# amzn/pecos

Measured on AMD Instinct MI355X. Metric: XLinear queries/sec @ beam=10 top-k=10; P@1 vs reference; 1/2/4/8 GPU, higher is better.
Workload: dtype f32; 1 GPU; amazon-670k synthetic x1.0: N=490000 D=135000 L=670091 tree=[2, 32, 512, 8192, 670091] nnz/row=75.4 beam=10 topk=10 pp=l3-hinge bias=1.0; parallelism=query-shard x1

## Files before the change

pecos_amd/csrc/xrl_abi.cpp:

```cpp
#include <algorithm>
#include <cstring>
#include <memory>
#include <mutex>

#include "xrl_host_pipeline.h"

namespace xrl {
thread_local std::string g_err;
thread_local bool g_has_err = false;
thread_local int g_device = 0;

void set_err(const std::string& s) { g_err = s; g_has_err = true; }

Model* as_model(void* p) {
    if (!p) fail("null model handle");
    return static_cast<Model*>(p);
}

void use_device(int dev) { XRL_HIP(hipSetDevice(dev)); }

void require_gpu() {
    int n = 0;
    if (hipGetDeviceCount(&n) != hipSuccess || n <= 0)
        fail("libxrl_amd: no HIP device visible -- this library has no CPU fallback");
}

void upload_x(const HostX& x, DevBuf& ptr, DevBuf& idx, DevBuf& val, QueriesDev& d) {
    if (!x.given) fail("null X");
    const uint64_t elems = x.elems();
    if (x.csr) {
        ptr.upload_raw(x.row_ptr, ((size_t)x.rows + 1) * 8);
        idx.upload_raw(x.col_idx, elems * 4);
    }
    val.upload_raw(x.val, elems * 4);
    d = device_view(x, ptr, idx, val);
}
}

using namespace xrl;

extern "C" {

const char* xrl_last_error(void) { return g_has_err ? g_err.c_str() : nullptr; }
void xrl_clear_error(void) { g_has_err = false; }
const char* xrl_version(void) { return "xrl_amd 0.1 (gfx950)"; }

int xrl_device_count(void) {
    int n = 0;
    if (hipGetDeviceCount(&n) != hipSuccess) return 0;
    return n;
}

int xrl_set_device(int device) {
    return guarded_value(-1, [&] { use_device(device); g_device = device; return 0; });
}

static void* load_handle(const char* model_path, int kind, int weight_matrix_type) {
    return guarded_value((void*)nullptr, [&]() -> void* {
        if (!model_path) fail("null model path");
        require_gpu();
        use_device(g_device);
        auto m = kind == 0 ? load_model_from_disk(model_path, weight_matrix_type) : load_mmap_model_from_disk(model_path);
        m->device = g_device; m->src_path = model_path; m->src_kind = kind;
        warm_handle(*m);
        return m.release();
    });
}

void* c_xlinear_load_model_from_disk_ext(const char* model_path, int weight_matrix_type) { return load_handle(model_path, 0, weight_matrix_type); }
void* c_xlinear_load_model_from_disk(const char* model_path) { return load_handle(model_path, 0, 2 ); }
void* c_xlinear_load_mmap_model_from_disk(const char* model_path, const bool) { return load_handle(model_path, 1, 2); }

void c_xlinear_compile_mmap_model(const char* model_path, const char* mmap_model_path) {
    guarded([&] {
        if (!model_path || !mmap_model_path) fail("null path");
        compile_mmap_model(model_path, mmap_model_path);
    });
}

void c_xlinear_destruct_model(void* ptr) {
    guarded([&] {
        if (!ptr) return;
        Model* m = static_cast<Model*>(ptr);
        (void)hipSetDevice(m->device);
        delete m;
    });
}

uint32_t c_xlinear_get_int_attr(void* ptr, const char* attr) {
    uint32_t v = 0;
    guarded([&] {
        Model& m = *as_model(ptr);
        if (!attr) fail("null attr");
        if (!std::strcmp(attr, "depth")) v = (uint32_t)m.layers.size();
        else if (!std::strcmp(attr, "nr_features")) v = m.nr_features;
        else if (!std::strcmp(attr, "nr_labels")) v = m.nr_labels;
        else if (!std::strcmp(attr, "nr_codes")) v = m.nr_codes;
        else if (!std::strcmp(attr, "device")) v = (uint32_t)m.device;
        else if (!std::strcmp(attr, "nr_pred_cols")) {
            const Layer& last = *m.layers.back();
            v = last.reordered ? last.c_rows : last.w_cols;
        }
        else if (!std::strcmp(attr, "nr_bucket_layers")) {
            for (auto& l : m.layers) v += l->dev.bucket ? 1u : 0u;
        }
        else if (!std::strcmp(attr, "nr_bitmap64_layers")) {
            for (auto& l : m.layers) v += l->dev.bitmap64 ? 1u : 0u;
        }
        else if (!std::strcmp(attr, "nr_dense_layers")) {
            for (auto& l : m.layers) v += l->dev.wd ? 1u : 0u;
        }
        else if (!std::strcmp(attr, "merged01")) v = m.layers[0]->dev.wd01 ? 1u : 0u;
        else if (!std::strcmp(attr, "nr_devices")) v = 1u + (uint32_t)m.replicas.size();
        else fail(std::string(attr) + " is not implemented in get_int_attr.");
    });
    return v;
}

int c_xlinear_get_layer_type(void* ptr, int layer_depth) {
    int v = -1;
    guarded([&] {
        Model& m = *as_model(ptr);
        if (layer_depth < 0 || (size_t)layer_depth >= m.layers.size()) fail("layer_depth out of range");
        v = m.weight_matrix_type;
    });
    return v;
}

void c_xlinear_predict_csr_f32(void* ptr, const ScipyCsrF32* input_x, const uint32_t overridden_beam_size,
                               const char* overridden_post_processor_str, const uint32_t overridden_only_topk,
                               const int , py_sparse_allocator_t pred_alloc) {
    guarded([&] { predict_host(ptr, HostX(input_x), overridden_beam_size, overridden_post_processor_str, overridden_only_topk, pred_alloc); });
}

void c_xlinear_predict_drm_f32(void* ptr, const ScipyDrmF32* input_x, const uint32_t overridden_beam_size,
                               const char* overridden_post_processor_str, const uint32_t overridden_only_topk,
                               const int , py_sparse_allocator_t pred_alloc) {
    guarded([&] { predict_host(ptr, HostX(input_x), overridden_beam_size, overridden_post_processor_str, overridden_only_topk, pred_alloc); });
}

int xrl_inspect_model(const char* model_path, uint64_t* out, uint32_t cap) {
    int depth = -1;
    guarded([&] {
        if (!model_path) fail("null model path");
        const std::string path(model_path);
        const JsonValue meta = parse_json_file(path + "/param.json");
        const JsonValue* dv = meta.get("depth");
        if (!dv || dv->type != JsonValue::NUMBER) fail(path + "/param.json: missing \"depth\"");
        const int d_n = (int)dv->num;
        for (int d = 0; d < d_n; ++d) {
            const std::string lp = path + "/" + std::to_string(d) + ".model";
            (void)parse_json_file(lp + "/param.json");
            HostCsc W, C;
            load_csc_npz(lp + "/W.npz", W);
            uint64_t c_rows = W.cols, c_cols = 1, c_nnz = W.cols;
            if (!(d == 0 && !file_exists(lp + "/C.npz"))) { load_csc_npz(lp + "/C.npz", C); c_rows = C.rows; c_cols = C.cols; c_nnz = C.nnz(); }
            const uint64_t rec[6] = {W.rows, W.cols, W.nnz(), c_rows, c_cols, c_nnz};
            for (int i = 0; i < 6; ++i) if (out && (uint32_t)(6 * d + i) < cap) out[6 * d + i] = rec[i];
        }
        depth = d_n;
    });
    return depth;
}

static void* queries_upload(void* model, const HostX& x) {
    return guarded_value((void*)nullptr, [&]() -> void* {
        Model& m = *as_model(model);
        use_device(m.device);
        auto q = std::make_unique<Queries>();
        QueriesDev d{};
        upload_x(x, q->ptr, q->idx, q->val, d);
        set_view(*q, m.device, d);
        return q.release();
    });
}
void* xrl_queries_upload_csr(void* model, const ScipyCsrF32* X) { return queries_upload(model, HostX(X)); }
void* xrl_queries_upload_drm(void* model, const ScipyDrmF32* X) { return queries_upload(model, HostX(X)); }

void* xrl_queries_from_device_csr(void* model, uint32_t rows, uint32_t cols, const uint64_t* d_row_ptr, const uint32_t* d_col_idx,
                                  const float* d_val, uint64_t nnz) {
    return guarded_value((void*)nullptr, [&]() -> void* {
        Model& m = *as_model(model);
        if (rows && (!d_row_ptr || (nnz && (!d_col_idx || !d_val)))) fail("xrl_queries_from_device_csr: null device pointer");
        auto q = std::make_unique<Queries>();
        set_view(*q, m.device, csr_view(rows, cols, d_row_ptr, d_col_idx, d_val, nnz));
        return q.release();
    });
}

void* xrl_queries_tfidf_device(void* model, uint32_t rows, uint32_t cols, const uint64_t* d_row_ptr, const uint32_t* d_col_idx,
                               const float* d_count, uint64_t nnz, const float* d_idf, int binary, int sublinear_tf, int norm_p, float* d_out,
                               void* hip_stream) {
    return guarded_value((void*)nullptr, [&]() -> void* {
        Model& m = *as_model(model);
        if (rows && (!d_row_ptr || (nnz && (!d_col_idx || !d_count)))) fail("xrl_queries_tfidf_device: null device pointer");
        use_device(m.device);
        auto q = std::make_unique<Queries>();
        if (!d_out) q->val.reserve(nnz * 4);
        float* dst = d_out ? d_out : q->val.as<float>();
        hipStream_t s = hip_stream ? static_cast<hipStream_t>(hip_stream) : m.stream;
        DevBuf d_err; d_err.reserve(4);
        XRL_HIP(hipMemsetAsync(d_err.p, 0, 4, s));
        launch_tfidf_weight(d_row_ptr, d_col_idx, d_count, d_idf, rows, cols, binary, sublinear_tf, norm_p, dst, s, 1, 0, d_err.as<uint32_t>());
        uint32_t err = 0;
        XRL_HIP(hipMemcpyAsync(&err, d_err.p, 4, hipMemcpyDeviceToHost, s));
        XRL_HIP(hipStreamSynchronize(s));
        if (err) fail("xrl_queries_tfidf_device: a column id outside [0, cols) (the reference's idx_idf.at() throws)");
        set_view(*q, m.device, csr_view(rows, cols, d_row_ptr, d_col_idx, dst, nnz));
        return q.release();
    });
}

void* xrl_queries_from_device_drm(void* model, uint32_t rows, uint32_t cols, const float* d_val) {
    return guarded_value((void*)nullptr, [&]() -> void* {
        Model& m = *as_model(model);
        if (rows && cols && !d_val) fail("xrl_queries_from_device_drm: null device pointer");
        auto q = std::make_unique<Queries>();
        set_view(*q, m.device, dense_view(rows, cols, d_val));
        return q.release();
    });
}

static void* concat_csr(void* model, uint32_t rows, uint32_t sparse_cols, const uint64_t* d_row_ptr, const uint32_t* d_col_idx, const float* d_val,
                        uint64_t nnz, uint32_t dense_cols, const float* d_emb, int normalize_emb, void* hip_stream) {
    Model& m = *as_model(model);
    if (rows && (!d_row_ptr || (nnz && (!d_col_idx || !d_val)) || (dense_cols && !d_emb))) fail("xrl_queries_concat_device: null device pointer");
    use_device(m.device);
    auto q = std::make_unique<Queries>();
    const uint64_t out_nnz = nnz + (uint64_t)rows * dense_cols;
    q->ptr.reserve(((size_t)rows + 1) * 8); q->idx.reserve(out_nnz * 4); q->val.reserve(out_nnz * 4);
    hipStream_t s = hip_stream ? static_cast<hipStream_t>(hip_stream) : m.stream;
    launch_concat_csr(d_row_ptr, d_col_idx, d_val, d_emb, rows, sparse_cols, dense_cols, normalize_emb, q->ptr.as<uint64_t>(), q->idx.as<uint32_t>(),
                      q->val.as<float>(), s);
    XRL_HIP(hipStreamSynchronize(s));
    set_own_csr(*q, m.device, rows, sparse_cols + dense_cols, out_nnz);
    return q.release();
}

void* xrl_queries_concat_device(void* model, uint32_t rows, uint32_t sparse_cols, const uint64_t* d_row_ptr, const uint32_t* d_col_idx,
                                const float* d_val, uint64_t nnz, uint32_t dense_cols, const float* d_emb, void* hip_stream) {
    return xrl_queries_concat_device_ex(model, rows, sparse_cols, d_row_ptr, d_col_idx, d_val, nnz, dense_cols, d_emb, 0, hip_stream);
}

void* xrl_queries_concat_device_ex(void* model, uint32_t rows, uint32_t sparse_cols, const uint64_t* d_row_ptr, const uint32_t* d_col_idx,
                                   const float* d_val, uint64_t nnz, uint32_t dense_cols, const float* d_emb, int normalize_emb, void* hip_stream) {
    return guarded_value((void*)nullptr, [&] {
        return concat_csr(model, rows, sparse_cols, d_row_ptr, d_col_idx, d_val, nnz, dense_cols, d_emb, normalize_emb, hip_stream);
    });
}

void* xrl_queries_concat_handle(void* model, void* queries, uint32_t dense_cols, const float* d_emb, int normalize_emb, void* hip_stream) {
    return guarded_value((void*)nullptr, [&] {
        if (!queries) fail("xrl_queries_concat_handle: null query handle");
        const QueriesDev& X = static_cast<Queries*>(queries)->dev;
        if (X.dense) fail("xrl_queries_concat_handle: the query handle must hold a CSR");
        return concat_csr(model, X.rows, X.cols, X.row_ptr, X.col_idx, X.val, X.nnz, dense_cols, d_emb, normalize_emb, hip_stream);
    });
}

int xrl_queries_info(void* queries, uint64_t* out4) {
    return guarded_value(-1, [&] {
        if (!queries || !out4) fail("null argument");
        const Queries* q = static_cast<const Queries*>(queries);
        out4[0] = q->dev.rows; out4[1] = q->dev.cols; out4[2] = q->dev.dense ? (uint64_t)q->dev.rows * q->dev.cols : q->dev.nnz; out4[3] = q->dev.dense ? 1 : 0;
        return 0;
    });
}

int xrl_queries_download(void* queries, uint64_t* row_ptr, uint32_t* col_idx, float* val) {
    return guarded_value(-1, [&] {
        if (!queries || !val) fail("null argument");
        const Queries* q = static_cast<const Queries*>(queries);
        XRL_HIP(hipSetDevice(q->device));
        XRL_HIP(hipDeviceSynchronize());
        if (q->dev.dense) {
            XRL_HIP(hipMemcpy(val, q->dev.val, (size_t)q->dev.rows * q->dev.cols * 4, hipMemcpyDeviceToHost));
        } else {
            if (!row_ptr || (q->dev.nnz && !col_idx)) fail("null argument");
            XRL_HIP(hipMemcpy(row_ptr, q->dev.row_ptr, ((size_t)q->dev.rows + 1) * 8, hipMemcpyDeviceToHost));
            if (q->dev.nnz) {
                XRL_HIP(hipMemcpy(col_idx, q->dev.col_idx, (size_t)q->dev.nnz * 4, hipMemcpyDeviceToHost));
                XRL_HIP(hipMemcpy(val, q->dev.val, (size_t)q->dev.nnz * 4, hipMemcpyDeviceToHost));
            }
        }
        return 0;
    });
}

void xrl_queries_free(void* queries) {
    guarded([&] {
        if (!queries) return;
        Queries* q = static_cast<Queries*>(queries);
        (void)hipSetDevice(q->device);
        delete q;
    });
}

static int predict_device_entry(const char* what, bool ranged, void* model, void* queries, uint32_t beam_size, const char* post_processor,
                                uint32_t only_topk, uint32_t* d_out_idx, float* d_out_val, uint32_t* d_out_cnt, uint32_t out_stride,
                                void* hip_stream, int sync, uint32_t row_begin = 0, uint32_t row_count = 0xFFFFFFFFu) {
    return guarded_value(-1, [&] {
        Model& m = *as_model(model);
        if (!queries || !d_out_idx || !d_out_val || !d_out_cnt) fail(std::string(what) + ": null argument");
        std::lock_guard<std::mutex> g(m.mu);
        use_device(m.device);
        const QueriesDev& X = static_cast<Queries*>(queries)->dev;
        PredictOpts o; o.beam_size = beam_size; o.only_topk = only_topk; o.post_processor = post_processor;
        if (ranged) o.reserve_rows = X.rows;
        predict_device(m, X, o, d_out_idx, d_out_val, d_out_cnt, out_stride, static_cast<hipStream_t>(hip_stream), sync != 0, row_begin, row_count);
        return 0;
    });
}

int xrl_predict_device(void* model, void* queries, uint32_t beam_size, const char* post_processor, uint32_t only_topk,
                       uint32_t* d_out_idx, float* d_out_val, uint32_t* d_out_cnt, uint32_t out_stride,
                       void* hip_stream, int sync) {
    return predict_device_entry("xrl_predict_device", false, model, queries, beam_size, post_processor, only_topk, d_out_idx, d_out_val, d_out_cnt, out_stride, hip_stream, sync);
}

int xrl_predict_device_rows(void* model, void* queries, uint32_t beam_size, const char* post_processor, uint32_t only_topk,
                            uint32_t* d_out_idx, float* d_out_val, uint32_t* d_out_cnt, uint32_t out_stride,
                            void* hip_stream, int sync, uint32_t row_begin, uint32_t row_count) {
    return predict_device_entry("xrl_predict_device_rows", true, model, queries, beam_size, post_processor, only_topk, d_out_idx, d_out_val, d_out_cnt, out_stride, hip_stream, sync, row_begin, row_count);
}

int xrl_ensemble_device(int device, uint32_t n_models, uint32_t rows, const uint32_t* const* d_idx, const float* const* d_val,
                        const uint32_t* const* d_cnt, const uint32_t* in_stride, int mode, const float* threshold, uint32_t only_topk,
                        uint32_t* d_out_idx, float* d_out_val, uint32_t* d_out_cnt, uint32_t out_stride, void* hip_stream, int sync) {
    return guarded_value(-1, [&] {
        const std::string what = "xrl_ensemble_device: ";
        if (!d_idx || !d_val || !d_cnt || !in_stride || !d_out_idx || !d_out_val || !d_out_cnt) fail(what + "null argument");
        if (n_models == 0 || n_models > (uint32_t)kEnsembleMaxModels) fail(what + "n_models must be 1.." + std::to_string(kEnsembleMaxModels) + ", got " + std::to_string(n_models));
        EnsembleArgs A{};
        uint64_t total = 0;
        for (uint32_t m = 0; m < n_models; ++m) {
            if (!d_idx[m] || !d_val[m] || !d_cnt[m]) fail(what + "null device pointer for model " + std::to_string(m));
            A.idx[m] = d_idx[m]; A.val[m] = d_val[m]; A.cnt[m] = d_cnt[m]; A.stride[m] = in_stride[m];
            total += in_stride[m];
        }
        if (total > kEnsembleMaxTotal) fail(what + "the input strides sum to " + std::to_string(total) + ", more than " + std::to_string(kEnsembleMaxTotal));
        if (mode != kEnsembleAverage && mode != kEnsembleFinish && mode != kEnsembleRankAverage) fail(what + "unknown mode " + std::to_string(mode));
        if (mode != kEnsembleFinish && (threshold || only_topk)) fail(what + "threshold and only_topk belong to mode finish");
        const uint64_t longest = mode == kEnsembleFinish && only_topk ? std::min<uint64_t>(total, only_topk) : total;
        if (out_stride < longest) fail(what + "out_stride " + std::to_string(out_stride) + " smaller than the longest possible row, " + std::to_string(longest));
        if (rows == 0) return 0;
        require_gpu();
        use_device(device);
        A.n_models = n_models; A.rows = rows; A.mode = mode;
        A.has_threshold = threshold ? 1 : 0; A.threshold = threshold ? *threshold : 0.0f; A.only_topk = only_topk;
        A.out_idx = d_out_idx; A.out_val = d_out_val; A.out_cnt = d_out_cnt; A.out_stride = out_stride;
        hipStream_t s = static_cast<hipStream_t>(hip_stream);
        void* mm = nullptr;
        if (mode == kEnsembleRankAverage) XRL_HIP(hipMallocAsync(&mm, sizeof(uint32_t), s));
        try { launch_ensemble(A, static_cast<uint32_t*>(mm), s); }
        catch (...) { if (mm) (void)hipFreeAsync(mm, s); throw; }
        if (mm) XRL_HIP(hipFreeAsync(mm, s));
        if (sync) XRL_HIP(hipStreamSynchronize(s));
        return 0;
    });
}

int xrl_predict_selected_device(void* model, void* queries, const char* post_processor, const uint32_t* d_sel_idx, const uint32_t* d_sel_cnt,
                                uint32_t sel_stride, uint32_t* d_out_idx, float* d_out_val, uint32_t* d_out_cnt, uint32_t out_stride,
                                uint32_t* d_status, void* hip_stream, int sync) {
    return guarded_value(-1, [&] {
        const std::string what = "xrl_predict_selected_device: ";
        if (!model || !queries || !d_sel_idx || !d_out_idx || !d_out_val || !d_out_cnt) fail(what + "null argument");
        Model& m = *as_model(model);
        const Queries& q = *static_cast<Queries*>(queries);
        if (sel_stride == 0 || sel_stride > kSelectMaxStride) fail(what + "sel_stride must be 1.." + std::to_string(kSelectMaxStride) + ", got " + std::to_string(sel_stride) + " (the host entry point serves longer rows)");
        if (out_stride < sel_stride) fail(what + "out_stride " + std::to_string(out_stride) + " smaller than sel_stride " + std::to_string(sel_stride));
        if (q.device != m.device) fail(what + "the queries live on device " + std::to_string(q.device) + ", the model on device " + std::to_string(m.device));
        std::lock_guard<std::mutex> g(m.mu);
        try { check_selected_inputs(m, q.dev); }
        catch (const Error& e) { fail(what + e.what()); }
        if (q.dev.rows == 0) return 0;
        use_device(m.device);
        predict_selected_device(m, q.dev, post_processor, d_sel_idx, d_sel_cnt, sel_stride, d_out_idx, d_out_val, d_out_cnt, out_stride, d_status,
                                static_cast<hipStream_t>(hip_stream), sync != 0);
        return 0;
    });
}

int xrl_predict_stats(void* model, void* queries, uint32_t beam_size, const char* post_processor, uint32_t only_topk,
                      double* stats_out, uint32_t stats_cap) {
    return guarded_value(-1, [&] {
        Model& m = *as_model(model);
        if (!queries || !stats_out) fail("xrl_predict_stats: null argument");
        if (stats_cap < kStatsPerLayer * m.layers.size()) fail("xrl_predict_stats: stats_out too small (need 8*depth doubles)");
        std::lock_guard<std::mutex> g(m.mu);
        if (m.constrained) fail("xrl_predict_stats: not available while an output constraint is set (the constrained route runs none of the counted kernels)");
        use_device(m.device);
        if (!m.ws) m.ws = std::make_unique<Workspace>();
        const QueriesDev& X = static_cast<Queries*>(queries)->dev;
        const uint32_t k = effective_topk(m, only_topk);
        Workspace& ws = *m.ws;
        ws.out_idx.reserve((size_t)X.rows * k * 4); ws.out_val.reserve((size_t)X.rows * k * 4); ws.out_cnt.reserve((size_t)X.rows * 4);
        PredictOpts o; o.beam_size = beam_size; o.only_topk = only_topk; o.post_processor = post_processor; o.stats_out = stats_out;
        const bool was = m.profiling; m.profiling = false;
        predict_device(m, X, o, ws.out_idx.as<uint32_t>(), ws.out_val.as<float>(), ws.out_cnt.as<uint32_t>(), k, m.stream, true);
        m.profiling = was;
        return 0;
    });
}

static int set_constraint_entry(const char* what, void* model, const uint32_t* labels, uint64_t n, bool on_device, void* hip_stream) {
    return guarded_value(-1, [&] {
        Model& m = *as_model(model);
        std::lock_guard<std::mutex> g(m.mu);
        use_device(m.device);
        set_output_constraint(m, labels, n, on_device, static_cast<hipStream_t>(hip_stream), what);
        return 0;
    });
}

int xrl_set_output_constraint(void* model, const uint32_t* labels, uint64_t n) {
    return set_constraint_entry("xrl_set_output_constraint", model, labels, n, false, nullptr);
}

int xrl_set_output_constraint_device(void* model, const uint32_t* d_labels, uint64_t n, void* hip_stream) {
    return set_constraint_entry("xrl_set_output_constraint_device", model, d_labels, n, true, hip_stream);
}

int xrl_clear_output_constraint(void* model) {
    return guarded_value(-1, [&] {
        Model& m = *as_model(model);
        std::lock_guard<std::mutex> g(m.mu);
        use_device(m.device);
        clear_output_constraint(m);
        return 0;
    });
}

int xrl_output_constraint_info(void* model, uint64_t* out, uint32_t cap) {
    return guarded_value(-1, [&] {
        Model& m = *as_model(model);
        std::lock_guard<std::mutex> g(m.mu);
        const uint32_t n = 1u + (uint32_t)m.layers.size();
        for (uint32_t i = 0; i < n && i < cap && out; ++i) {
            if (i == 0) { out[0] = m.constrained ? 1 : 0; continue; }
            const Layer& L = *m.layers[i - 1];
            out[i] = L.view.active ? L.view.kept : L.n_children;
        }
        return (int)n;
    });
}

int xrl_debug_output_constraint_view(void* model, uint32_t layer, uint32_t* chunk_col_out, uint64_t chunk_col_cap, uint32_t* perm_inv_out, uint64_t perm_inv_cap) {
    return guarded_value(-1, [&] {
        Model& m = *as_model(model);
        if (layer >= m.layers.size()) fail("xrl_debug_output_constraint_view: layer out of range");
        std::lock_guard<std::mutex> g(m.mu);
        const Layer& L = *m.layers[layer];
        if (!L.view.active) return 0;
        use_device(m.device);
        XRL_HIP(hipDeviceSynchronize());
        const uint64_t n_cc = std::min<uint64_t>(chunk_col_cap, (uint64_t)L.dev.n_parents + 1), n_pi = std::min<uint64_t>(perm_inv_cap, L.view.kept);
        if (chunk_col_out && n_cc) XRL_HIP(hipMemcpy(chunk_col_out, L.view.d_chunk_col.p, n_cc * 4, hipMemcpyDeviceToHost));
        if (perm_inv_out && n_pi) XRL_HIP(hipMemcpy(perm_inv_out, L.view.d_perm_inv.p, n_pi * 4, hipMemcpyDeviceToHost));
        return 1;
    });
}

uint32_t xrl_effective_topk(void* model, uint32_t only_topk) {
    return guarded_value(0u, [&] { return effective_topk(*as_model(model), only_topk); });
}

void xrl_profile_enable(void* model, int enable) { guarded([&] { as_model(model)->profiling = enable != 0; }); }
void xrl_profile_reset(void* model) { guarded([&] { Model& m = *as_model(model); resolve_profile(m); m.profile.clear(); }); }
uint32_t xrl_profile_get(void* model, xrl_profile_rec_t* out, uint32_t cap) {
    uint32_t n = 0;
    guarded([&] {
        Model& m = *as_model(model);
        resolve_profile(m);
        n = (uint32_t)m.profile.size();
        for (uint32_t i = 0; i < n && i < cap && out; ++i) {
            std::memset(&out[i], 0, sizeof(out[i]));
            std::strncpy(out[i].name, m.profile[i].name.c_str(), sizeof(out[i].name) - 1);
            out[i].layer = m.profile[i].layer; out[i].launches = m.profile[i].launches;
            out[i].ms = m.profile[i].ms;
        }
    });
    return n;
}

uint32_t xrl_debug_split_chunk(const uint64_t* cum, uint32_t n, uint64_t limit) {
    return guarded_value(0u, [&] { if (!cum) fail("null cum"); return split_chunk(cum, n, limit); });
}

uint64_t xrl_debug_layout_rows(const uint32_t* rptr, uint32_t nrows, int align, uint32_t* ext_out) {
    return guarded_value((uint64_t)0, [&] { if (!rptr) fail("null rptr"); return layout_tile_rows(rptr, nrows, align != 0, ext_out); });
}

uint32_t xrl_debug_host_batches(const uint64_t* row_ptr, uint32_t rows, uint32_t cols, int host_batch_mb, uint32_t* rb_out, uint32_t cap) {
    return guarded_value(0u, [&] {
        HostX x; x.given = true; x.csr = row_ptr != nullptr; x.rows = rows; x.cols = cols; x.row_ptr = row_ptr;
        const std::vector<uint32_t> rb = plan_row_batches(x, host_batch_mb, staged_upload(x, 1));
        for (size_t i = 0; i < rb.size() && i < cap && rb_out; ++i) rb_out[i] = rb[i];
        return (uint32_t)rb.size();
    });
}

#define XRL_OPT(name) {#name, &Model::Options::name}
static const struct { const char* name; int Model::Options::*field; } kIntOptions[] = {
    XRL_OPT(k1_group), XRL_OPT(sort_min_tiles), XRL_OPT(sort_rest), XRL_OPT(sort_rest_min), XRL_OPT(prune_mid), XRL_OPT(leaf_fuse), XRL_OPT(tile_rows),
    XRL_OPT(k2_big_min_k), XRL_OPT(qsort), XRL_OPT(qsort_min_parents), XRL_OPT(qsort_min_rows), XRL_OPT(presence), XRL_OPT(adaptive), XRL_OPT(prune),
    XRL_OPT(host_pipeline), XRL_OPT(host_batch_mb), XRL_OPT(host_register), XRL_OPT(overlap_min_rows),
    XRL_OPT(dense_layers), XRL_OPT(k1q_fuse), XRL_OPT(k1g_first), XRL_OPT(k1g_min_items), XRL_OPT(k1g_variant),
    XRL_OPT(k1_wpb), XRL_OPT(k1_lds_pad), XRL_OPT(k1_ablate),
};
#undef XRL_OPT

static void set_option_one(Model& m, const char* key, int64_t value) {
    if (!std::strcmp(key, "max_batch_rows")) { m.opt.max_batch_rows = value; return; }
    if (!std::strcmp(key, "reserve_rows")) {
        if (value < 0 || value > 0x7FFFFFFF) fail("reserve_rows: expected 0 .. 2^31-1");
        std::lock_guard<std::mutex> g(m.mu);
        use_device(m.device);
        if (!m.ws) m.ws = std::make_unique<Workspace>();
        reserve_outputs(m, (uint32_t)value, effective_topk(m, 0));
        return;
    }
    for (const auto& o : kIntOptions)
        if (!std::strcmp(key, o.name)) { m.opt.*o.field = (int)value; if (o.field == &Model::Options::adaptive) m.fb.restage(); return; }
    fail(std::string("unknown option ") + key);
}

int xrl_set_option(void* model, const char* key, int64_t value) {
    return guarded_value(-1, [&] {
        Model& m = *as_model(model);
        if (!key) fail("null key");
        if (!std::strcmp(key, "devices")) {
            if (value < 1 || value > 64) fail("devices: expected 1..64");
            if (m.src_kind < 0 && value > 1) fail("devices: only models loaded from a folder can be replicated");
            std::lock_guard<std::mutex> g(m.mu);
            if (m.constrained && value > 1) fail("devices: the handle carries an output constraint, which replicas do not share (xrl_clear_output_constraint first)");
            int ndev = 0;
            XRL_HIP(hipGetDeviceCount(&ndev));
            m.replicas.clear();
            for (int64_t i = 1; i < value; ++i) {
                const int dev = (m.device + (int)i) % std::max(1, ndev);
                use_device(dev);
                std::unique_ptr<Model> r = m.src_kind == 0 ? load_model_from_disk(m.src_path, m.weight_matrix_type) : load_mmap_model_from_disk(m.src_path);
                r->device = dev;
                r->opt = m.opt;
                m.replicas.push_back(std::move(r));
            }
            use_device(m.device);
        } else {
            set_option_one(m, key, value);
            for (auto& r : m.replicas) set_option_one(*r, key, value);
        }
        return 0;
    });
}

void xrl_debug_k1_phases(unsigned long long* out8, int reset) { guarded([&] { k1_phase_read(out8, reset != 0); }); }

uint32_t xrl_layer_info(void* model, uint32_t layer, uint64_t* out, uint32_t cap) {
    uint32_t n = 0;
    guarded([&] {
        Model& m = *as_model(model);
        if (layer >= m.layers.size()) fail("xrl_layer_info: layer out of range");
        const Layer& L = *m.layers[layer];
        const uint64_t rec[12] = {
            (uint64_t)(L.dev.bucket ? 1 : (L.dev.bitmap64 ? 2 : 0)), L.bk_levels, (uint64_t)(L.dev.wd ? 1 : 0), 1ull << L.dev.d_gp_log2,
            L.dev.d_ld, L.n_tiles, L.nnz, L.dense_bytes, L.w_rows, L.n_children, L.max_tile_cols, L.device_bytes};
        n = 12;
        for (uint32_t i = 0; i < n && i < cap && out; ++i) out[i] = rec[i];
    });
    return n;
}

uint64_t xrl_model_device_bytes(void* model) {
    return guarded_value((uint64_t)0, [&] { return as_model(model)->device_bytes(); });
}

}
```

pecos_amd/csrc/xrl_k0.hip:

```cpp
#include <hip/hip_runtime.h>

#include "xrl_kernels.h"
#include "xrl_items.h"

namespace xrl {

__global__ void __launch_bounds__(256)
k0_prolongate(const uint32_t* __restrict__ chunk_col, const uint32_t* __restrict__ ptile,
              const TileDesc* __restrict__ tiles, uint32_t nrows, uint32_t beam_in, uint32_t item_ranks, uint32_t TT, uint32_t cand_stride,
              int implicit_root, const uint32_t* __restrict__ p_idx, const float* __restrict__ p_val,
              const uint32_t* __restrict__ p_cnt, uint32_t p_stride, uint32_t* __restrict__ cand_off,
              uint32_t* __restrict__ ncand, ItemDesc* __restrict__ items, const uint64_t* __restrict__ x_row_ptr) {
    const uint32_t q = blockIdx.x * 256u + threadIdx.x;
    if (q >= nrows) return;
    uint64_t xb = 0; uint32_t xl = 0;
    if (x_row_ptr) { xb = x_row_ptr[q]; xl = (uint32_t)(x_row_ptr[q + 1] - xb); }
    const uint32_t cnt = implicit_root ? 1u : min(p_cnt[q], beam_in);
    uint32_t off = 0;
    for (uint32_t j = 0; j < beam_in; ++j) {
        ItemDesc* it = items + ((size_t)q * item_ranks + j) * TT;
        uint32_t nt = 0;
        if (j < cnt) {
            const uint32_t parent = implicit_root ? 0u : p_idx[(size_t)q * p_stride + j];
            const float ps = implicit_root ? 1.0f : p_val[(size_t)q * p_stride + j];
            const uint32_t cb = chunk_col[parent], t0 = ptile[parent];
            nt = ptile[parent + 1] - t0;
            cand_off[(size_t)q * beam_in + j] = off;
            if (j < item_ranks)
                for (uint32_t tt = 0; tt < nt; ++tt)
                    it[tt] = make_item(q, t0 + tt, q * cand_stride + off + (tiles[t0 + tt].col_begin - cb), ps, xb, xl);
            off += chunk_col[parent + 1] - cb;
        }
        if (j < item_ranks) for (uint32_t tt = nt; tt < TT; ++tt) it[tt] = make_item(q, kNoTile, 0u, 0.f, 0, 0u);
    }
    ncand[q] = off;
}

void launch_k0_prolongate(const LayerDev& L, const LayerPlan& P, const QueriesDev& X, BeamDev prev, uint32_t* cand_off,
                          uint32_t* ncand, void* items, hipStream_t s, uint32_t item_ranks) {
    if (P.nrows == 0) return;
    if ((uint64_t)P.nrows * P.cand_stride > 0xFFFFFFFFull) fail("k0: candidate buffer exceeds 2^32 floats; lower max_batch_rows");
    hipLaunchKernelGGL(k0_prolongate, dim3((P.nrows + 255) / 256), dim3(256), 0, s, L.chunk_col, L.ptile, L.tiles,
                       P.nrows, P.beam_in, std::min(item_ranks, P.beam_in), L.max_tiles_per_parent, P.cand_stride, P.implicit_root, prev.idx, prev.val,
                       prev.cnt, prev.stride, cand_off, ncand, static_cast<ItemDesc*>(items),
                       X.dense ? nullptr : X.row_ptr + P.row0);
    XRL_LAUNCH_CHECK();
}
size_t k0_item_bytes() { return sizeof(ItemDesc); }

__global__ void __launch_bounds__(256)
k0b_remaining(const uint32_t* __restrict__ chunk_col, const uint32_t* __restrict__ ptile, const TileDesc* __restrict__ tiles,
              uint32_t nrows, uint32_t beam_in, uint32_t first_rank, uint32_t end_rank, uint32_t cand_stride, const uint32_t* __restrict__ p_idx,
              const float* __restrict__ p_val, const uint32_t* __restrict__ p_cnt, uint32_t p_stride, const uint32_t* __restrict__ cand_off,
              const uint32_t* __restrict__ done, ItemDesc* __restrict__ items, uint32_t* __restrict__ n_items,
              const uint64_t* __restrict__ x_row_ptr) {
    const uint32_t q = blockIdx.x * 256u + threadIdx.x;
    const int lane = threadIdx.x & 63;
    const bool live = q < nrows && !done[q];
    const uint32_t cnt = live ? min(min(p_cnt[q], beam_in), end_rank) : 0u;
    uint32_t n = 0;
    for (uint32_t j = first_rank; j < cnt; ++j) { const uint32_t parent = p_idx[(size_t)q * p_stride + j]; n += ptile[parent + 1] - ptile[parent]; }
    uint32_t incl = n;
#pragma unroll
    for (int d = 1; d < 64; d <<= 1) { const uint32_t y = (uint32_t)__shfl_up((int)incl, d, 64); if (lane >= d) incl += y; }
    const uint32_t total = (uint32_t)__shfl((int)incl, 63, 64);
    uint32_t base = 0;
    if (lane == 63 && total) base = atomicAdd(n_items, total);
    base = (uint32_t)__shfl((int)base, 63, 64) + incl - n;
    if (n == 0) return;
    uint64_t xb = 0; uint32_t xl = 0;
    if (x_row_ptr) { xb = x_row_ptr[q]; xl = (uint32_t)(x_row_ptr[q + 1] - xb); }
    for (uint32_t j = first_rank; j < cnt; ++j) {
        const uint32_t parent = p_idx[(size_t)q * p_stride + j];
        const float ps = p_val[(size_t)q * p_stride + j];
        const uint32_t cb = chunk_col[parent], t0 = ptile[parent], nt = ptile[parent + 1] - t0;
        const uint32_t off = cand_off[(size_t)q * beam_in + j];
        for (uint32_t tt = 0; tt < nt; ++tt)
            items[base++] = make_item(q, t0 + tt, q * cand_stride + off + (tiles[t0 + tt].col_begin - cb), ps, xb, xl);
    }
}

void launch_k0b_remaining(const LayerDev& L, const LayerPlan& P, const QueriesDev& X, BeamDev prev, const uint32_t* cand_off, const uint32_t* done,
                          uint32_t first_rank, void* items, uint32_t* n_items, hipStream_t s, uint32_t end_rank) {
    if (P.nrows == 0) return;
    XRL_HIP(hipMemsetAsync(n_items, 0, 4, s));
    hipLaunchKernelGGL(k0b_remaining, dim3((P.nrows + 255) / 256), dim3(256), 0, s, L.chunk_col, L.ptile, L.tiles, P.nrows, P.beam_in, first_rank, end_rank,
                       P.cand_stride, prev.idx, prev.val, prev.cnt, prev.stride, cand_off, done, static_cast<ItemDesc*>(items), n_items,
                       X.dense ? nullptr : X.row_ptr + P.row0);
    XRL_LAUNCH_CHECK();
}

}
```

pecos_amd/csrc/xrl_k1.hip:

```cpp
#include <hip/hip_runtime.h>

#include "xrl_device.h"
#include "xrl_kernels.h"
#include "xrl_items.h"

namespace xrl {

struct K1Args {
    LayerDev L;
    QueriesDev X;
    const ItemDesc* items;
    const uint32_t* n_items;
    float* cand;
    uint64_t n_slots;
    uint32_t row0, acc_stride;
    int pp_kind, pp_p, first_layer;
    int bias_first;
    int ablate;
    uint32_t lds_per_wave;
    uint32_t n_vblocks;
    unsigned long long* phase;
    uint32_t* fb_out;
};

template <int G, int PPC, class ACC>
__device__ __forceinline__ void k1_epilogue(const K1Args& a, const ItemDesc& it, const TileDesc& td, int lig, ACC&& acc_at,
                                            bool add_bias) {
    if (it.tile == kNoTile || (a.ablate & 16)) return;
    float* __restrict__ out = a.cand + it.out_off;
    const float* __restrict__ bp = a.L.bias_prod + td.col_begin;
    if (a.ablate & 8) {
        for (uint32_t c = lig; c < td.ncols; c += G) {
            const float acc = add_bias ? __fadd_rn(acc_at(c), bp[c]) : acc_at(c);
            out[c] = a.first_layer ? acc : pp_combine(a.pp_kind, acc, it.pscore);
        }
        return;
    }
    for (uint32_t c = lig; c < td.ncols; c += G) out[c] = finish_score<PPC>(acc_at(c), add_bias, bp + c, a.pp_kind, a.pp_p, a.first_layer, it.pscore);
}

struct __attribute__((packed, aligned(4))) RowExt { uint32_t start, end; };

template <int G, int NS> struct K1Cfg {
    static constexpr int W = 64 / G;
#ifndef XRL_K1_FEAT
#define XRL_K1_FEAT 64
#endif
    static constexpr int U = (G >= 16) ? XRL_K1_FEAT / G : 8;
    static constexpr int H = (G > 32) ? 2 * G : 64;
    static constexpr int UH = H * NS;
#ifndef XRL_K1_P
#define XRL_K1_P 4
#endif
#ifndef XRL_K1_CLAMP
#define XRL_K1_CLAMP 1
#endif
#ifndef XRL_K1_NB
#define XRL_K1_NB 2
#endif
    static constexpr int P = XRL_K1_P;
    static constexpr int NB = XRL_K1_NB;
    static constexpr int TAIL = (2 * NB - 1) * P;
    static constexpr size_t lds_bytes(uint32_t acc_stride) {
        return (size_t)W * (UH + TAIL) * 8 + (size_t)W * H * 8 + (size_t)W * (acc_stride + G) * 4;
    }
};

#ifndef XRL_K1_WPE
#define XRL_K1_WPE 5
#endif
template <int G, int NS, int PPC, bool DENSE, int LK>
__global__ void __launch_bounds__(256) __attribute__((amdgpu_waves_per_eu(XRL_K1_WPE, 8))) k1_kernel(K1Args a) {
    constexpr int W = K1Cfg<G, NS>::W, H = K1Cfg<G, NS>::H, UH = K1Cfg<G, NS>::UH, P = K1Cfg<G, NS>::P, U = K1Cfg<G, NS>::U,
                  NB = K1Cfg<G, NS>::NB, TAIL = K1Cfg<G, NS>::TAIL;
    extern __shared__ __attribute__((aligned(16))) unsigned char smem_all[];
    const uint32_t wave = threadIdx.x >> 6;
    const uint32_t vblock = blockIdx.x * (blockDim.x >> 6) + wave;
    if (vblock >= a.n_vblocks) return;
    unsigned char* smem = smem_all + (size_t)wave * a.lds_per_wave;
    uint2* uq = reinterpret_cast<uint2*>(smem);
    uint2* hq = reinterpret_cast<uint2*>(uq + W * (UH + TAIL));
    float* acc = reinterpret_cast<float*>(hq + W * H);
    const uint32_t acc_item = a.acc_stride + G;

    const int lane = threadIdx.x & 63;
    const int grp = lane / G, lig = lane % G;
#ifdef XRL_K1_PHASE_PROF
    const bool prof = a.phase != nullptr;
    unsigned long long t_last = prof ? __builtin_readcyclecounter() : 0ull, t_ph[5] = {0, 0, 0, 0, 0};
    auto tick = [&](int ph) { if (prof) { const unsigned long long t = __builtin_readcyclecounter(); t_ph[ph] += t - t_last; t_last = t; } };
#else
    auto tick = [](int) {};
#endif
    ItemDesc it;
    if (!fetch_item<W>(a.items, a.n_items, a.n_slots, a.fb_out, vblock, grp, lane, it)) return;
    const bool active = it.tile != kNoTile;
    TileDesc td{};
    uint64_t xe = 0, cur = 0;
    if (active) {
        td = a.L.tiles[it.tile];
        cur = it.x_begin; xe = it.x_begin + it.x_len;
    }
    const uint32_t* __restrict__ rp = a.L.row_ext + td.rowptr_base;
    const Entry* __restrict__ ent = a.L.entries + td.ent_base;
    float* __restrict__ my_acc = acc + (size_t)grp * acc_item;
    uint2* __restrict__ my_hq = hq + (size_t)grp * H;
    uint2* __restrict__ my_uq = uq + (size_t)grp * (UH + TAIL);
    const uint32_t dummy = a.acc_stride + (uint32_t)lig;
    if (DENSE || a.bias_first) {
        const float* __restrict__ bp = a.L.bias_prod + td.col_begin;
        for (uint32_t c = lig; c < td.ncols; c += G) my_acc[c] = a.L.has_bias ? bp[c] : 0.0f;
    } else if (!(a.ablate & 32)) {
        for (uint32_t c = lig; c < td.ncols; c += G) my_acc[c] = 0.0f;
    }
    wave_sync_lds();
    if (a.ablate & 2) cur = xe;

    const BmWord* __restrict__ bm = a.L.bitmap + (LK != 0 ? 0ull : (uint64_t)(active ? it.tile : 0u) * a.L.nwords);
    const BmWord64* __restrict__ bm64 = a.L.bitmap64 + (LK != 2 ? 0ull : (uint64_t)(active ? it.tile : 0u) * a.L.nwords64);
    const uint32_t* __restrict__ bkt = LK == 1 ? a.L.bucket + (uint64_t)(active ? it.tile : 0u) * (a.L.bk_n + 1u) : nullptr;
    const uint32_t* __restrict__ ridx_t = a.L.row_idx + td.rowptr_base;
    const uint64_t xlast = xe > cur ? xe - 1 : 0;
    uint32_t nh = 0;
    tick(0);

    auto drain = [&]() {
        if (a.ablate & 4) { nh = 0; return; }
        tick(1);
        wave_sync_lds();
        uint32_t nu = 0;
        for (uint32_t h0 = 0; __any(h0 < nh); h0 += G) {
            const uint32_t h = h0 + lig;
            const bool ok = h < nh;
            const uint2 hv = my_hq[ok ? h : 0u];
            const bool need = ok && (LK != 2 || DENSE || (hv.y >> 25) == 0x7Fu);
            const uint32_t s = need ? ((LK == 2 && !DENSE) ? (hv.y & 0x1FFFFFFu) : hv.y) : 0u;
            const uint32_t rl = rp[s];
            const uint32_t rx = need ? rl : hv.y;
            const uint32_t rs = rx & 0x1FFFFFFu;
            const uint32_t len = ok ? (rx >> 25) + 1u : 0u;
            uint32_t cnt = (NS == 1) ? (len ? 1u : 0u) : min((len + G - 1) / G, (uint32_t)NS);
            uint32_t incl = cnt;
            if (G > 1) {
#pragma unroll
                for (int d = 1; d < G; d <<= 1) { const uint32_t y = __shfl_up(incl, d, G); if (lig >= d) incl += y; }
            }
            const uint32_t base = nu + incl - cnt;
#pragma unroll
            for (int k = 0; k < NS; ++k)
                if ((uint32_t)k < cnt) {
                    const uint32_t n_k = (k == NS - 1) ? len - (uint32_t)k * G : min(len - (uint32_t)k * G, (uint32_t)G);
                    my_uq[base + k] = make_uint2(hv.x, (rs + (uint32_t)k * G) | (n_k << 25));
                }
            nu += (G > 1) ? __shfl(incl, G - 1, G) : incl;
        }
        uint32_t nu_max = nu;
#pragma unroll
        for (int d = G; d < 64; d <<= 1) nu_max = max(nu_max, (uint32_t)__shfl_xor((int)nu_max, d, 64));
        nu_max = __builtin_amdgcn_readfirstlane(nu_max);
        for (uint32_t j = nu + lig; j < nu_max + (uint32_t)TAIL; j += G) my_uq[j] = make_uint2(0u, 0u);
        wave_sync_lds();
        tick(2);
        const uint2* __restrict__ uqp = my_uq;
        struct Batch { uint32_t xv[P], cn[P]; Entry e[P]; };
        auto load_batch = [&](const uint2* q, Batch& B) {
            uint32_t st[P];
#pragma unroll
            for (int p = 0; p < P; ++p) { const uint2 d = q[p]; B.xv[p] = d.x; st[p] = d.y & 0x1FFFFFFu; B.cn[p] = d.y >> 25; }
#pragma unroll
            for (int p = 0; p < P; ++p) {
#if XRL_K1_CLAMP
                B.e[p] = ent[st[p] + ((uint32_t)lig < B.cn[p] ? (uint32_t)lig : 0u)];
#else
                B.e[p] = ent[st[p] + (uint32_t)lig];
#endif
            }
        };
        auto apply_batch = [&](const Batch& B) {
#pragma unroll
            for (int p = 0; p < P; ++p) {
                const float v = __uint_as_float(B.xv[p]);
                const uint32_t ci = (uint32_t)lig < B.cn[p] ? B.e[p].col : dummy;
                my_acc[ci] = __fadd_rn(my_acc[ci], __fmul_rn(v, B.e[p].val));
                wave_sync_lds();
            }
        };
        Batch ring[NB];
#pragma unroll
        for (int b = 0; b < NB - 1; ++b) load_batch(uqp + b * P, ring[b]);
        for (uint32_t i0 = 0; i0 < nu_max; i0 += NB * P) {
#pragma unroll
            for (int b = 0; b < NB; ++b) {
                load_batch(uqp + (b + NB - 1) * P, ring[(b + NB - 1) % NB]);
                apply_batch(ring[b]);
            }
            uqp += NB * P;
        }
        nh = 0;
        tick(3);
    };

    if (DENSE) {
        const float* __restrict__ xd = a.X.val + ((uint64_t)a.row0 + it.q) * a.X.cols;
        const uint32_t* __restrict__ ridx = a.L.row_idx + td.rowptr_base;
        uint32_t nr = active ? td.nrows : 0u;
        if (active && td.bias_slot != kNoBias) nr -= 1;
        for (uint32_t s0 = 0; __any(s0 < nr); s0 += H) {
            for (uint32_t j = lig; j < (uint32_t)H; j += G) {
                const uint32_t sidx = s0 + j;
                const bool ok = sidx < nr;
                const uint32_t f = ridx[ok ? sidx : 0u];
                const float xval = xd[f < a.X.cols ? f : 0u];
                if (ok) my_hq[j] = make_uint2(__float_as_uint(f < a.X.cols ? xval : 0.0f), sidx);
            }
            nh = s0 < nr ? min((uint32_t)H, nr - s0) : 0u;
            drain();
        }
        k1_epilogue<G, PPC>(a, it, td, lig, [&](uint32_t c) { return my_acc[c]; }, false);
        return;
    }
    uint32_t skip = 0;
    while (__any(cur < xe)) {
        bool overflow = false;
        {
            uint32_t f[U]; float v[U];
            load_features<G, U>(a.X.col_idx, a.X.val, cur, xe, xlast, a.L.w_rows, lig, f, v);
            bool hit[U]; uint32_t slot[U];
            if (LK == 0) {
                if (a.ablate & 1) {
#pragma unroll
                    for (int u = 0; u < U; ++u) f[u] = 0xFFFFFFFFu;
                }
                probe_bitmap32<U>(bm, f, hit, slot, [](const BmWord& w, uint32_t before) { return w.rank + before; });
            } else if (LK == 2) {
                probe_bitmap64<U>(bm64, f, hit, slot, [](const BmWord64& w, uint32_t before) { return before == 0u ? w.ext0 : (0xFE000000u | (w.rank + before)); });
            } else {
                uint32_t hi[U];
#pragma unroll
                for (int u = 0; u < U; ++u) {
                    const bool inr = f[u] != 0xFFFFFFFFu;
                    const RowExt be = *reinterpret_cast<const RowExt*>(bkt + (inr ? (f[u] >> a.L.bk_shift) : 0u));
                    slot[u] = be.start; hi[u] = inr ? be.end : be.start;
                }
                for (uint32_t lv = a.L.bk_levels; lv > 0; --lv) {
                    const uint32_t stp = 1u << (lv - 1);
#pragma unroll
                    for (int u = 0; u < U; ++u) {
                        const uint32_t np = slot[u] + stp;
                        const bool in = np < hi[u];
                        const uint32_t r = ridx_t[in ? np : slot[u]];
                        slot[u] = (in && r <= f[u]) ? np : slot[u];
                    }
                }
#pragma unroll
                for (int u = 0; u < U; ++u) hit[u] = slot[u] < hi[u] && ridx_t[slot[u]] == f[u];
            }
            overflow = queue_hits<G, U, H>(hit, v, slot, my_hq, grp, lig, nh, skip, cur, xe);
        }
        if (__any(overflow)) drain();
    }
    drain();
    k1_epilogue<G, PPC>(a, it, td, lig, [&](uint32_t c) { return my_acc[c]; }, a.L.has_bias != 0 && !a.bias_first);
#ifdef XRL_K1_PHASE_PROF
    if (prof) {
        tick(4);
        if (lane == 0) { for (int i = 0; i < 5; ++i) atomicAdd(&a.phase[i], t_ph[i]); atomicAdd(&a.phase[5], 1ull); }
    }
#endif
}

template <class KERNEL>
static void launch_k1_any(KERNEL kernel, K1Args a, int W, size_t lds_wave, const K1Tune& tune, hipStream_t s) {
    lds_wave = (lds_wave + (size_t)std::max(0, tune.lds_pad) + 15) & ~(size_t)15;
    int wpb = (tune.wpb == 2 || tune.wpb == 4) ? tune.wpb : 1;
    while (wpb > 1 && lds_wave * wpb > 160 * 1024) wpb >>= 1;
    const size_t lds = lds_wave * wpb;
    if (lds > 160 * 1024) fail("k1: LDS request exceeds 160 KiB");
    if (lds > 48 * 1024)
        XRL_HIP(hipFuncSetAttribute(reinterpret_cast<const void*>(kernel), hipFuncAttributeMaxDynamicSharedMemorySize, (int)lds));
    const uint64_t vblocks = (a.n_slots + W - 1) / W;
    const uint64_t blocks = (vblocks + wpb - 1) / wpb;
    if (vblocks > 0x7FFFFFFFull) fail("k1: grid too large; lower max_batch_rows");
    a.lds_per_wave = (uint32_t)lds_wave; a.n_vblocks = (uint32_t)vblocks;
    hipLaunchKernelGGL(kernel, dim3((uint32_t)blocks), dim3(64 * wpb), lds, s, a);
    XRL_LAUNCH_CHECK();
}

static unsigned long long* g_phase_buf = nullptr;
unsigned long long* k1_phase_buffer() {
    if (!g_phase_buf) { XRL_HIP(hipMalloc(&g_phase_buf, 8 * 8)); XRL_HIP(hipMemset(g_phase_buf, 0, 64)); }
    return g_phase_buf;
}
void k1_phase_read(unsigned long long out[8], bool reset) {
    XRL_HIP(hipDeviceSynchronize());
    XRL_HIP(hipMemcpy(out, k1_phase_buffer(), 64, hipMemcpyDeviceToHost));
    if (reset) XRL_HIP(hipMemset(g_phase_buf, 0, 64));
}

int k1_auto_group(const LayerDev& L, const Layer& host, int dense) {
    (void)host; (void)dense;
    if (L.max_tile_cols <= 8) return 8;
    if (L.max_tile_cols <= 16) return 16;
    return 32;
}

void launch_k1(const LayerDev& L, const LayerPlan& P, const QueriesDev& X, const void* items, const uint32_t* n_items,
               float* cand, int group, hipStream_t s) {
    if (P.nrows == 0) return;
    if ((P.tune.tile_rows >= 2 || (P.tune.tile_rows == 1 && !n_items)) && P.tune.ablate == 0 && k1t_serves(L, X)) { launch_k1t(L, P, X, items, n_items, cand, s); return; }
    K1Args a;
    a.L = L; a.X = X; a.items = static_cast<const ItemDesc*>(items); a.n_items = n_items; a.cand = cand;
    a.n_slots = (uint64_t)P.nrows * P.beam_in * L.max_tiles_per_parent;
    a.row0 = P.row0; a.pp_kind = P.pp.kind; a.pp_p = P.pp.p; a.first_layer = P.first_layer; a.bias_first = P.bias_first;
    a.acc_stride = L.max_tile_cols | 1u;
    const int ablate = P.tune.ablate;
    a.ablate = ablate & 0xFF;
    a.phase = ((ablate & 64) && ((ablate >> 8) == 0 || (ablate >> 8) == P.layer + 1)) ? k1_phase_buffer() : nullptr;
    a.fb_out = (n_items && P.fb_host && P.layer >= 0 && P.layer < kFbLayers) ? P.fb_host + fb_items_word(P.layer) : nullptr;
    const int ppc = pp_class(P.pp);
#define XRL_K1_PP(GG, NN, DD, LL) do { if (ppc) launch_k1_any(&k1_kernel<GG, NN, 1, DD, LL>, a, 64 / GG, lds, P.tune, s); else launch_k1_any(&k1_kernel<GG, NN, 0, DD, LL>, a, 64 / GG, lds, P.tune, s); } while (0)
#define XRL_K1(GG, NN) do { \
        const size_t lds = K1Cfg<GG, NN>::lds_bytes(a.acc_stride); \
        if (X.dense) XRL_K1_PP(GG, NN, true, 0); \
        else if (L.bucket) XRL_K1_PP(GG, NN, false, 1); \
        else if (L.bitmap64) XRL_K1_PP(GG, NN, false, 2); \
        else XRL_K1_PP(GG, NN, false, 0); } while (0)
    if (group < 1 || group > 64 || (group & (group - 1))) fail("k1: lanes-per-item must be a power of two in [1, 64]");
    auto max_ns = [](int g) { return g < 8 ? 1u : (g == 32 ? 4u : 2u); };
    auto units = [&](int g) { return (L.max_tile_cols + (uint32_t)g - 1) / (uint32_t)g; };
    while (group < 64 && units(group) > max_ns(group)) group <<= 1;
    const uint32_t ns = units(group);
    switch (group) {
    case 1: XRL_K1(1, 1); break;
    case 2: XRL_K1(2, 1); break;
    case 4: XRL_K1(4, 1); break;
    case 8: if (ns <= 1) XRL_K1(8, 1); else XRL_K1(8, 2); break;
    case 16: if (ns <= 1) XRL_K1(16, 1); else XRL_K1(16, 2); break;
    case 32: if (ns <= 1) XRL_K1(32, 1); else if (ns == 2) XRL_K1(32, 2); else if (ns == 3) XRL_K1(32, 3); else XRL_K1(32, 4); break;
    default: if (ns <= 1) XRL_K1(64, 1); else XRL_K1(64, 2); break;
    }
#undef XRL_K1
#undef XRL_K1_PP
}

}
```

pecos_amd/csrc/xrl_k1t.hip:

```cpp
#include <hip/hip_runtime.h>

#include <cfloat>
#include <cmath>

#include "xrl_device.h"
#include "xrl_kernels.h"
#include "xrl_items.h"

namespace xrl {

namespace {

struct K1TArgs {
    LayerDev L;
    QueriesDev X;
    const ItemDesc* items;
    const uint32_t* n_items;
    float* cand;
    uint64_t n_slots;
    int pp_kind, pp_p, first_layer, bias_first;
    uint32_t n_vblocks;
    uint32_t* fb_out;
    uint32_t wt_bytes;
    const uint32_t* p_cnt; const float* p_val; uint32_t p_stride, beam_in;
    const uint32_t* xok; const uint32_t* perm_inv;
    uint32_t* out_idx; float* out_val; uint32_t* out_cnt; uint32_t* done;
    uint32_t out_stride, k;
    int mult;
    const uint32_t* p_idx; const uint64_t* x_row_ptr;
    uint32_t cand_stride; uint32_t* cand_off; uint32_t* ncand;
};

template <int NR> struct RowVec;
template <> struct RowVec<1> { float v[1]; };
template <> struct alignas(8) RowVec<2> { float v[2]; };
template <> struct RowVec<3> { float v[3]; };
template <> struct alignas(16) RowVec<4> { float v[4]; };

typedef uint32_t u32x2 __attribute__((ext_vector_type(2)));
typedef uint32_t u32x3 __attribute__((ext_vector_type(3)));
typedef uint32_t u32x4 __attribute__((ext_vector_type(4)));
template <int NR> __device__ __forceinline__ RowVec<NR> row_load_buf(__amdgpu_buffer_rsrc_t rs, uint32_t voff);
template <> __device__ __forceinline__ RowVec<1> row_load_buf<1>(__amdgpu_buffer_rsrc_t rs, uint32_t voff) { return __builtin_bit_cast(RowVec<1>, __builtin_amdgcn_raw_buffer_load_b32(rs, (int)voff, 0, 0)); }
template <> __device__ __forceinline__ RowVec<2> row_load_buf<2>(__amdgpu_buffer_rsrc_t rs, uint32_t voff) { return __builtin_bit_cast(RowVec<2>, __builtin_amdgcn_raw_buffer_load_b64(rs, (int)voff, 0, 0)); }
template <> __device__ __forceinline__ RowVec<3> row_load_buf<3>(__amdgpu_buffer_rsrc_t rs, uint32_t voff) {
    const auto t = __builtin_amdgcn_raw_buffer_load_b96(rs, (int)voff, 0, 0);
    RowVec<3> r; r.v[0] = __uint_as_float(t[0]); r.v[1] = __uint_as_float(t[1]); r.v[2] = __uint_as_float(t[2]); return r;
}
template <> __device__ __forceinline__ RowVec<4> row_load_buf<4>(__amdgpu_buffer_rsrc_t rs, uint32_t voff) { return __builtin_bit_cast(RowVec<4>, __builtin_amdgcn_raw_buffer_load_b128(rs, (int)voff, 0, 0)); }

template <int G, int NR, int PPC, int LK, bool BUF, bool SEL>
__global__ void __launch_bounds__(256) __attribute__((amdgpu_waves_per_eu(5, 8))) k1t_kernel(K1TArgs a) {
    constexpr int W = 64 / G, H = 64, U = (G >= 16) ? 64 / G : 8, UNR = 8, STRIDE = G * NR;
    __shared__ uint2 hq_all[4 * W * (H + UNR)];
    const uint32_t wave = threadIdx.x >> 6;
    const uint32_t vblock = blockIdx.x * 4u + wave;
    if (vblock >= a.n_vblocks) return;
    const int lane = threadIdx.x & 63;
    const int grp = lane / G, lig = lane % G;
    uint2* __restrict__ my_hq = hq_all + ((size_t)wave * W + grp) * (H + UNR);

    auto derive_item = [&](uint64_t q) {
        const uint32_t cnt = min(a.p_cnt[q], a.beam_in);
        const uint32_t parent = cnt ? a.p_idx[q * a.p_stride] : 0u;
        const float ps = a.p_val[q * a.p_stride];
        const uint64_t xb = a.x_row_ptr[q];
        const uint32_t xl = (uint32_t)(a.x_row_ptr[q + 1] - xb);
        const uint32_t t0 = a.L.ptile[parent], t1 = a.L.ptile[parent + 1];
        return make_item((uint32_t)q, (cnt && t1 > t0) ? t0 : kNoTile, (uint32_t)q * a.cand_stride, ps, xb, xl);
    };
    ItemDesc it;
    if (SEL && !a.items && !a.n_items) {
        const uint64_t slot = (uint64_t)vblock * W + grp;
        it = slot < a.n_slots ? derive_item(slot) : make_item(0u, kNoTile, 0u, 0.f, 0, 0u);
    } else if (!fetch_item<W>(a.items, a.n_items, a.n_slots, a.fb_out, vblock, grp, lane, it)) return;
    bool active = it.tile != kNoTile;
    TileDesc td{};
    uint64_t xe = 0, cur = 0, wbase = 0;
    if (active) {
        td = a.L.tiles[it.tile];
        wbase = a.L.wt_base[it.tile];
        cur = it.x_begin; xe = it.x_begin + it.x_len;
    }
    const char* __restrict__ wrow = reinterpret_cast<const char*>(a.L.wt + (BUF ? 0ull : wbase) + (uint32_t)(NR * lig));
    const uint32_t tbase = BUF ? (uint32_t)(wbase * 4ull) : 0u;
    const uint32_t lane_off = (uint32_t)(NR * lig * 4);
    const __amdgpu_buffer_rsrc_t wrs = __builtin_amdgcn_make_buffer_rsrc(const_cast<float*>(a.L.wt), 0, (int)(BUF ? a.wt_bytes : 0u), 0x00020000);
    const uint32_t pad_off = tbase + td.nrows * (uint32_t)(STRIDE * 4);
    float acc[NR];
    {
        const float* __restrict__ bp = a.L.bias_prod + td.col_begin;
#pragma unroll
        for (int k = 0; k < NR; ++k) {
            const uint32_t c = (uint32_t)(NR * lig + k);
            acc[k] = (a.bias_first && a.L.has_bias && c < td.ncols) ? bp[c] : 0.0f;
        }
    }
    const BmWord* __restrict__ bm = a.L.bitmap + (LK != 0 ? 0ull : (uint64_t)(active ? it.tile : 0u) * a.L.nwords);
    const BmWord64* __restrict__ bm64 = a.L.bitmap64 + (LK != 2 ? 0ull : (uint64_t)(active ? it.tile : 0u) * a.L.nwords64);
    const uint64_t xlast = xe > cur ? xe - 1 : 0;
    uint32_t nh = 0;
    bool nonfin = false;

    auto drain = [&](auto exact_tag) {
        constexpr bool EX = decltype(exact_tag)::value;
        wave_sync_lds();
        uint32_t nh_max = nh;
#pragma unroll
        for (int d = G; d < 64; d <<= 1) nh_max = max(nh_max, (uint32_t)__shfl_xor((int)nh_max, d, 64));
        nh_max = __builtin_amdgcn_readfirstlane(nh_max);
        for (uint32_t j = nh + (uint32_t)lig; j < ((nh_max + UNR - 1u) & ~(uint32_t)(UNR - 1)); j += G) my_hq[j] = make_uint2(0u, pad_off);
        wave_sync_lds();
#pragma unroll 1
        for (uint32_t h0 = 0; h0 < nh_max; h0 += UNR) {
            uint2 hv[UNR];
            RowVec<NR> w[UNR];
#pragma unroll
            for (int u = 0; u < UNR; ++u) hv[u] = my_hq[h0 + u];
#pragma unroll
            for (int u = 0; u < UNR; ++u) w[u] = BUF ? row_load_buf<NR>(wrs, hv[u].y + lane_off) : *reinterpret_cast<const RowVec<NR>*>(wrow + hv[u].y);
#pragma unroll
            for (int u = 0; u < UNR; ++u) {
                const float x = __uint_as_float(hv[u].x);
#pragma unroll
                for (int k = 0; k < NR; ++k) {
                    const float s = __fadd_rn(acc[k], __fmul_rn(x, w[u].v[k]));
                    acc[k] = (EX && __float_as_uint(w[u].v[k]) == kMissing) ? acc[k] : s;
                }
            }
        }
        nh = 0;
    };
    auto drain_any = [&]() {
        if (nonfin) drain(std::true_type{}); else drain(std::false_type{});
        nonfin = false;
    };

    uint32_t skip = 0;
    while (__any(cur < xe)) {
        bool overflow = false;
        {
            uint32_t f[U]; float v[U];
            load_features<G, U>(a.X.col_idx, a.X.val, cur, xe, xlast, a.L.w_rows, lig, f, v);
            bool nf = false;
#pragma unroll
            for (int u = 0; u < U; ++u) nf |= (cur + (uint64_t)(u * G + lig) < xe) & ((__float_as_uint(v[u]) & 0x7F800000u) == 0x7F800000u);
            nonfin = nonfin || __any(nf);
            bool hit[U]; uint32_t off[U];
            if (LK == 0) probe_bitmap32<U>(bm, f, hit, off, [&](const BmWord& w, uint32_t before) { return tbase + (w.rank + before) * (uint32_t)(STRIDE * 4); });
            else probe_bitmap64<U>(bm64, f, hit, off, [&](const BmWord64& w, uint32_t before) { return tbase + (w.rank + before) * (uint32_t)(STRIDE * 4); });
            overflow = queue_hits<G, U, H>(hit, v, off, my_hq, grp, lig, nh, skip, cur, xe);
        }
        if (__any(overflow)) drain_any();
    }
    drain_any();

    if constexpr (SEL) {
        static_assert(G == 32, "the selecting epilogue ranks one item per half-wavefront");
        int lane_e = lane;
        asm volatile("" : "+v"(lane_e));
        const int grp = lane_e >> 5, lig = lane_e & 31;
        const uint64_t slot = (uint64_t)vblock * W + grp;
        const bool qv = slot < a.n_slots;
        const uint64_t q = qv ? slot : 0;
        if constexpr (NR == 4) {
            it = a.items ? a.items[q] : derive_item(q);
            active = qv && it.tile != kNoTile;
            td = a.L.tiles[active ? it.tile : 0u];
        }
        const uint32_t pc = a.p_cnt[q], xok = a.xok[q];
        const float ps_next = a.p_val[q * a.p_stride + 1u];
        const float* __restrict__ bp = a.L.bias_prod + td.col_begin;
        const bool add_bias = a.L.has_bias != 0 && !a.bias_first;
        uint32_t key[NR], sb[NR];
#pragma unroll
        for (int k = 0; k < NR; ++k) {
            const uint32_t c = (uint32_t)(NR * lig + k);
            key[k] = 0u; sb[k] = 0u;
            if (active && c < td.ncols) {
                const float v = finish_score<PPC>(acc[k], add_bias, bp + c, a.pp_kind, a.pp_p, a.first_layer, it.pscore);
                sb[k] = __float_as_uint(v); key[k] = score_key(v);
            }
        }
        const bool limited = min(pc, a.beam_in) > 1u;
        const uint32_t thr = score_key(a.mult ? fmaxf(ps_next, 0.0f) : ps_next);
        uint32_t c_lo = 0, c_hi = 0;
#pragma unroll
        for (int k = 0; k < NR; ++k) {
            const unsigned long long b = __ballot(key[k] >= thr);
            c_lo += (uint32_t)__popc((uint32_t)b); c_hi += (uint32_t)__popc((uint32_t)(b >> 32));
        }
        const bool d = !limited || (xok != 0u && ps_next == ps_next && (grp ? c_hi : c_lo) >= a.k);
        if (!a.items && __any(qv && !d)) {
            const uint32_t cnt = min(pc, a.beam_in);
            const bool mine = qv && !d && (uint32_t)lig < cnt;
            uint32_t wd = 0;
            if (mine) { const uint32_t pj = a.p_idx[q * a.p_stride + (uint32_t)lig]; wd = a.L.chunk_col[pj + 1] - a.L.chunk_col[pj]; }
            uint32_t incl = wd;
#pragma unroll
            for (int s = 1; s < 32; s <<= 1) { const uint32_t y = (uint32_t)__shfl_up((int)incl, s, 32); if (lig >= s) incl += y; }
            const uint32_t total = (uint32_t)__shfl((int)incl, 31, 32);
            if (mine) a.cand_off[q * a.beam_in + (uint32_t)lig] = incl - wd;
            if (qv && !d && lig == 0) a.ncand[q] = total;
        }
        if (active && !d) {
            float* __restrict__ out = a.cand + it.out_off;
#pragma unroll
            for (int k = 0; k < NR; ++k) { const uint32_t c = (uint32_t)(NR * lig + k); if (c < td.ncols) out[c] = __uint_as_float(sb[k]); }
        }
        uint32_t osb, ops, kk_lo, kk_hi;
        halfwave_topk_extract<NR>(key, sb, a.k, lane_e, osb, ops, kk_lo, kk_hi);
        const uint32_t kk = grp ? kk_hi : kk_lo;
        if (qv) {
            if ((uint32_t)lig < kk) {
                uint32_t child = td.col_begin + ops;
                if (a.perm_inv) child = a.perm_inv[child];
                a.out_idx[q * a.out_stride + (uint32_t)lig] = child;
                a.out_val[q * a.out_stride + (uint32_t)lig] = __uint_as_float(osb);
            }
            if (lig == 0) { a.out_cnt[q] = kk; a.done[q] = d ? 1u : 0u; }
        }
        return;
    }
    if (!active) return;
    float* __restrict__ out = a.cand + it.out_off;
    const float* __restrict__ bp = a.L.bias_prod + td.col_begin;
    const bool add_bias = a.L.has_bias != 0 && !a.bias_first;
#pragma unroll
    for (int k = 0; k < NR; ++k) {
        const uint32_t c = (uint32_t)(NR * lig + k);
        if (c < td.ncols) out[c] = finish_score<PPC>(acc[k], add_bias, bp + c, a.pp_kind, a.pp_p, a.first_layer, it.pscore);
    }
}

__global__ void __launch_bounds__(256)
tile_rows_kernel(const TileDesc* __restrict__ tiles, const uint32_t* __restrict__ row_ext, const Entry* __restrict__ entries,
                 const uint64_t* __restrict__ wt_base, uint32_t stride, uint32_t* __restrict__ wt) {
    const TileDesc td = tiles[blockIdx.x];
    uint32_t* __restrict__ dst = wt + wt_base[blockIdx.x];
    const uint32_t* __restrict__ ext = row_ext + td.rowptr_base;
    const Entry* __restrict__ ent = entries + td.ent_base;
    const uint32_t sub = threadIdx.x >> 5, l = threadIdx.x & 31u;
    for (uint32_t r = sub; r < td.nrows; r += 8u) {
        const uint32_t e = ext[r], start = e & 0x1FFFFFFu, len = (e >> 25) + 1u;
        for (uint32_t i = l; i < len; i += 32u) {
            const Entry x = ent[start + i];
            const uint32_t b = __float_as_uint(x.val);
            dst[(uint64_t)r * stride + x.col] = b == kMissing ? 0u : b;
        }
    }
}

}

void k1t_shape(uint32_t max_tile_cols, int& g, int& nr) {
    g = max_tile_cols <= 8 ? 8 : max_tile_cols <= 16 ? 16 : 32;
    nr = (int)((max_tile_cols + (uint32_t)g - 1) / (uint32_t)g);
    if (nr < 1) nr = 1;
}

void launch_tile_rows(const LayerDev& L, uint64_t total_floats, uint32_t* wt, hipStream_t s) {
    XRL_HIP(hipMemsetD32Async(reinterpret_cast<hipDeviceptr_t>(wt), (int)kMissing, total_floats, s));
    if (L.n_tiles) {
        hipLaunchKernelGGL(tile_rows_kernel, dim3(L.n_tiles), dim3(256), 0, s, L.tiles, L.row_ext, L.entries, L.wt_base, L.wt_stride, wt);
        XRL_LAUNCH_CHECK();
    }
}

bool k1t_serves(const LayerDev& L, const QueriesDev& X) { return L.wt != nullptr && !X.dense && (L.bitmap || L.bitmap64) && !L.bucket; }

bool k1t_selects(const LayerDev& L, const LayerPlan& P, const QueriesDev& X) {
    int g, nr;
    k1t_shape(L.max_tile_cols, g, nr);
    return k1t_serves(L, X) && P.tune.tile_rows >= 1 && P.tune.ablate == 0 && L.max_tiles_per_parent == 1 && g == 32 && nr <= 4 &&
           P.k >= 1 && P.k <= kTopkExtractMaxK && P.beam_in >= 2 && !P.implicit_root && !P.first_layer && k2_wave_path(P);
}

void launch_k1t(const LayerDev& L, const LayerPlan& P, const QueriesDev& X, const void* items, const uint32_t* n_items, float* cand, hipStream_t s,
                const K1TSelect* sel) {
    if (P.nrows == 0) return;
    K1TArgs a{};
    a.L = L; a.X = X; a.items = static_cast<const ItemDesc*>(items); a.n_items = n_items; a.cand = cand;
    a.n_slots = sel ? (uint64_t)P.nrows : (uint64_t)P.nrows * P.beam_in * L.max_tiles_per_parent;
    a.pp_kind = P.pp.kind; a.pp_p = P.pp.p; a.first_layer = P.first_layer; a.bias_first = P.bias_first;
    a.fb_out = (n_items && P.fb_host && P.layer >= 0 && P.layer < kFbLayers) ? P.fb_host + fb_items_word(P.layer) : nullptr;
    int g, nr;
    k1t_shape(L.max_tile_cols, g, nr);
    if ((uint32_t)(g * nr) != L.wt_stride || nr > 4) fail("k1t: the layer's tile rows were laid out for another shape");
    const uint64_t vblocks = (a.n_slots + (uint64_t)(64 / g) - 1) / (uint64_t)(64 / g);
    if (vblocks > 0x7FFFFFFFull) fail("k1t: grid too large; lower max_batch_rows");
    a.n_vblocks = (uint32_t)vblocks;
    const int ppc = pp_class(P.pp);
    const int lk = L.bitmap64 ? 2 : 0;
    const bool buf = L.wt_bytes != 0 && L.wt_bytes < 0xFFFFFF00ull;
    a.wt_bytes = buf ? (uint32_t)L.wt_bytes : 0u;
    if (sel) {
        if (n_items || !k1t_selects(L, P, X)) fail("k1t: the selecting epilogue does not serve this launch");
        if (!sel->done || !sel->xok) fail("k1t: bound pruning needs the done and the per-query guard flags");
        a.p_cnt = sel->prev.cnt; a.p_val = sel->prev.val; a.p_stride = sel->prev.stride; a.beam_in = P.beam_in;
        a.xok = sel->xok; a.perm_inv = L.perm_inv;
        a.out_idx = sel->out.idx; a.out_val = sel->out.val; a.out_cnt = sel->out.cnt; a.done = sel->done;
        a.out_stride = sel->out.stride; a.k = P.k;
        a.mult = (P.pp.kind == PP_SIGMOID || P.pp.kind == PP_LP_HINGE) ? 1 : 0;
        if (!items) {
            if (!sel->cand_off || !sel->ncand || P.beam_in > 32u) fail("k1t: the launch cannot derive its items");
            if ((uint64_t)P.nrows * P.cand_stride > 0xFFFFFFFFull) fail("k1t: candidate buffer exceeds 2^32 floats; lower max_batch_rows");
            a.p_idx = sel->prev.idx; a.x_row_ptr = X.row_ptr + P.row0; a.cand_stride = P.cand_stride; a.cand_off = sel->cand_off; a.ncand = sel->ncand;
        }
    }
    const dim3 grid((a.n_vblocks + 3u) / 4u), block(256);
#define XRL_K1T_L(GG, NN, BB, SS) do { \
        if (ppc) { if (lk) hipLaunchKernelGGL((k1t_kernel<GG, NN, 1, 2, BB, SS>), grid, block, 0, s, a); else hipLaunchKernelGGL((k1t_kernel<GG, NN, 1, 0, BB, SS>), grid, block, 0, s, a); } \
        else     { if (lk) hipLaunchKernelGGL((k1t_kernel<GG, NN, 0, 2, BB, SS>), grid, block, 0, s, a); else hipLaunchKernelGGL((k1t_kernel<GG, NN, 0, 0, BB, SS>), grid, block, 0, s, a); } } while (0)
#define XRL_K1T(GG, NN) do { if (buf) XRL_K1T_L(GG, NN, true, false); else XRL_K1T_L(GG, NN, false, false); } while (0)
#define XRL_K1T_S(NN) do { if (sel) { if (buf) XRL_K1T_L(32, NN, true, true); else XRL_K1T_L(32, NN, false, true); } else XRL_K1T(32, NN); } while (0)
    if (g == 8) XRL_K1T(8, 1);
    else if (g == 16) XRL_K1T(16, 1);
    else if (nr == 1) XRL_K1T_S(1);
    else if (nr == 2) XRL_K1T_S(2);
    else if (nr == 3) XRL_K1T_S(3);
    else XRL_K1T_S(4);
#undef XRL_K1T_S
#undef XRL_K1T
#undef XRL_K1T_L
    XRL_LAUNCH_CHECK();
}

}
```

pecos_amd/csrc/xrl_k2.hip:

```cpp
#include <hip/hip_runtime.h>

#include "xrl_device.h"
#include "xrl_kernels.h"

namespace xrl {

struct K2Args {
    const uint32_t* chunk_col;
    const uint32_t* perm_inv;
    const uint32_t* p_idx; const uint32_t* p_cnt; uint32_t p_stride;
    const uint32_t* cand_off; const uint32_t* ncand; const float* cand;
    uint32_t* out_idx; float* out_val; uint32_t* out_cnt;
    uint32_t nrows, beam_in, cand_stride, k, out_stride;
    int implicit_root;
    const float* p_val;
    int mult;
    uint32_t rank_limit;
    uint32_t* done;
    const uint32_t* skip_done;
    const uint32_t* xok;
};

__device__ __forceinline__ uint32_t k2_child_id(const K2Args& a, uint64_t q, uint32_t pos) {
    uint32_t parent = 0, off = 0;
    if (!a.implicit_root) {
        const uint32_t cnt = min(a.p_cnt[q], a.beam_in);
        uint32_t jj = 0;
        for (uint32_t j = 1; j < cnt; ++j) if (a.cand_off[q * a.beam_in + j] <= pos) jj = j; else break;
        off = a.cand_off[q * a.beam_in + jj];
        parent = a.p_idx[q * a.p_stride + jj];
    }
    const uint32_t child = a.chunk_col[parent] + (pos - off);
    return a.perm_inv ? a.perm_inv[child] : child;
}

__global__ void __launch_bounds__(64) k2_topk_reg(K2Args a) {
    const uint64_t q = blockIdx.x;
    const int lane = threadIdx.x;
    const uint32_t n = a.ncand[q], k = a.k;
    const float* __restrict__ cv = a.cand + q * a.cand_stride;
    float lv = -INFINITY, th = -INFINITY;
    uint32_t lp = 0, m = 0;
    constexpr int KB = 4;
    const uint32_t nlast = n ? n - 1 : 0;
    for (uint32_t base0 = 0; base0 < n; base0 += 64 * KB) {
        float vb[KB];
#pragma unroll
        for (int b = 0; b < KB; ++b) { const uint32_t p = base0 + b * 64 + lane; vb[b] = cv[p < n ? p : nlast]; }
#pragma unroll
        for (int b = 0; b < KB; ++b) {
            const uint32_t base = base0 + b * 64;
            const uint32_t p = base + lane;
            const bool valid = p < n;
            const float v = vb[b];
            unsigned long long mask = __ballot(valid && (m < k || v > th));
            while (mask) {
                const int l = __ffsll((long long)mask) - 1;
                mask &= mask - 1;
                const float vv = __shfl(v, l);
                if (m == k && !(vv > th)) continue;
                const int r = __popcll(__ballot((uint32_t)lane < m && lv >= vv));
                const float uv = __shfl_up(lv, 1);
                const uint32_t up = __shfl_up(lp, 1);
                if (lane > r) { lv = uv; lp = up; }
                else if (lane == r) { lv = vv; lp = base + l; }
                if (m < k) ++m;
                th = (m == k) ? __shfl(lv, (int)k - 1) : -INFINITY;
            }
        }
    }
    if ((uint32_t)lane < m) {
        a.out_idx[q * a.out_stride + lane] = k2_child_id(a, q, lp);
        a.out_val[q * a.out_stride + lane] = lv;
    }
    if (lane == 0) a.out_cnt[q] = m;
}

__global__ void __launch_bounds__(64) k2_topk_lds(K2Args a) {
    extern __shared__ __attribute__((aligned(16))) unsigned char smem[];
    float* lv = reinterpret_cast<float*>(smem);
    uint32_t* lp = reinterpret_cast<uint32_t*>(lv + a.k);
    const uint64_t q = blockIdx.x;
    const int lane = threadIdx.x;
    const uint32_t n = a.ncand[q], k = a.k;
    const float* __restrict__ cv = a.cand + q * a.cand_stride;
    float th = -INFINITY;
    uint32_t m = 0;
    for (uint32_t base = 0; base < n; base += 64) {
        const uint32_t p = base + lane;
        const bool valid = p < n;
        const float v = valid ? cv[p] : 0.f;
        unsigned long long mask = __ballot(valid && (m < k || v > th));
        while (mask) {
            const int l = __ffsll((long long)mask) - 1;
            mask &= mask - 1;
            const float vv = __shfl(v, l);
            if (m == k && !(vv > th)) continue;
            uint32_t r = 0;
            for (uint32_t i0 = 0; i0 < m; i0 += 64) {
                const uint32_t i = i0 + lane;
                r += (uint32_t)__popcll(__ballot(i < m && lv[i] >= vv));
            }
            const uint32_t e = (m < k) ? m : k - 1;
            for (uint32_t hi = e; hi > r;) {
                const uint32_t lo = (hi - r > 64) ? hi - 64 : r;
                const uint32_t i = lo + lane;
                const bool mv = i < hi;
                float tv = 0.f; uint32_t tp = 0;
                if (mv) { tv = lv[i]; tp = lp[i]; }
                wave_sync_lds();
                if (mv) { lv[i + 1] = tv; lp[i + 1] = tp; }
                wave_sync_lds();
                hi = lo;
            }
            if (lane == 0) { lv[r] = vv; lp[r] = base + l; }
            wave_sync_lds();
            if (m < k) ++m;
            th = (m == k) ? lv[k - 1] : -INFINITY;
        }
    }
    wave_sync_lds();
    for (uint32_t i = lane; i < m; i += 64) {
        a.out_idx[q * a.out_stride + i] = k2_child_id(a, q, lp[i]);
        a.out_val[q * a.out_stride + i] = lv[i];
    }
    if (lane == 0) a.out_cnt[q] = m;
}

template <int NS>
__global__ void __launch_bounds__(256) k2_topk_wave(K2Args a) {
    __shared__ uint2 sc_all[4 * 64];
    const int lane = threadIdx.x & 63;
    const uint32_t wave = __builtin_amdgcn_readfirstlane(threadIdx.x >> 6);
    const uint32_t q32 = blockIdx.x * 4u + wave;
    if (q32 >= a.nrows) return;
    const uint64_t q = q32;
    if (a.skip_done && a.skip_done[q]) return;
    uint32_t n = min(a.ncand[q], (uint32_t)(64 * NS));
    const uint32_t bcnt0 = a.implicit_root ? 1u : min(a.p_cnt[q], a.beam_in);
    const uint32_t rl = min(a.rank_limit, a.beam_in - 1u);
    const uint32_t lim_off = a.rank_limit ? a.cand_off[q * a.beam_in + rl] : 0u;
    const float ps_next = a.rank_limit ? a.p_val[q * a.p_stride + rl] : 0.0f;
    const bool limited = a.rank_limit != 0u && bcnt0 > a.rank_limit;
    if (limited) n = min(n, lim_off);
    const float* __restrict__ cv = a.cand + q * a.cand_stride;
    const uint32_t slast = a.cand_stride - 1u;
    const uint32_t bcnt = a.implicit_root ? 1u : min(a.p_cnt[q], a.beam_in);
    const bool lane_beam = !a.implicit_root && bcnt <= 64u;
    uint32_t b_off = 0xFFFFFFFFu, b_par = 0u, b_cc = 0u;
    if (lane_beam && (uint32_t)lane < bcnt) { b_off = a.cand_off[q * a.beam_in + lane]; b_par = a.p_idx[q * a.p_stride + lane]; b_cc = a.chunk_col[b_par]; }
    uint32_t key[NS], sbits[NS], pos[NS];
#pragma unroll
    for (int r = 0; r < NS; ++r) {
        const uint32_t p = (uint32_t)r * 64u + (uint32_t)lane;
        const float v = cv[min(p, slast)];
        sbits[r] = __float_as_uint(v); pos[r] = p;
        key[r] = p < n ? score_key(v) : 0u;
    }
    if (a.done) {
        bool d = true;
        if (limited) d = a.xok[q] != 0u && ps_next == ps_next && wave_count_ge<NS>(key, score_key(a.mult ? fmaxf(ps_next, 0.0f) : ps_next)) >= a.k;
        if (lane == 0) a.done[q] = d ? 1u : 0u;
    }
    uint32_t rank, sb, pp;
    const uint32_t kk = wave_topk<NS>(key, sbits, pos, a.k, sc_all + wave * 64u, lane, rank, sb, pp);
    uint32_t child;
    if (lane_beam) {
        uint32_t jj = 0;
        for (uint32_t j = 1; j < bcnt; ++j) jj = ((uint32_t)__builtin_amdgcn_readlane((int)b_off, (int)j) <= pp) ? j : jj;
        const uint32_t off = (uint32_t)__shfl((int)b_off, (int)jj, 64), cc = (uint32_t)__shfl((int)b_cc, (int)jj, 64);
        child = cc + (pp - off);
        if ((uint32_t)lane < kk && a.perm_inv) child = a.perm_inv[child];
    } else {
        child = (uint32_t)lane < kk ? k2_child_id(a, q, pp) : 0u;
    }
    if ((uint32_t)lane < kk) {
        a.out_idx[q * a.out_stride + rank] = child;
        a.out_val[q * a.out_stride + rank] = __uint_as_float(sb);
    }
    if (lane == 0) a.out_cnt[q] = kk;
}

size_t k2_max_k() { return (160 * 1024) / 8; }

bool k2_wave_path(const LayerPlan& P) { return P.k <= 64 && P.cand_stride <= 64u * 32u; }

void launch_k2_topk(const LayerDev& L, const LayerPlan& P, BeamDev prev, const uint32_t* cand_off,
                    const uint32_t* ncand, const float* cand, BeamDev out, hipStream_t s, uint32_t rank_limit, uint32_t limited_cands,
                    uint32_t* done, const uint32_t* skip_done, const uint32_t* xok) {
    if (P.nrows == 0) return;
    K2Args a;
    a.p_val = prev.val; a.rank_limit = rank_limit; a.done = done; a.skip_done = skip_done; a.xok = xok;
    if (done && !xok) fail("k2: bound pruning needs the per-query guard flags");
    a.mult = (P.pp.kind == PP_SIGMOID || P.pp.kind == PP_LP_HINGE) ? 1 : 0;
    if ((rank_limit || done || skip_done) && !k2_wave_path(P)) fail("k2: bound pruning needs the register top-k path");
    a.chunk_col = L.chunk_col; a.perm_inv = L.perm_inv;
    a.p_idx = prev.idx; a.p_cnt = prev.cnt; a.p_stride = prev.stride;
    a.cand_off = cand_off; a.ncand = ncand; a.cand = cand;
    a.out_idx = out.idx; a.out_val = out.val; a.out_cnt = out.cnt;
    a.nrows = P.nrows; a.beam_in = P.beam_in; a.cand_stride = P.cand_stride; a.k = P.k; a.out_stride = out.stride;
    a.implicit_root = P.implicit_root;
    if (P.k == 0) fail("k2: only_topk / beam_size resolved to 0");
    if (!rank_limit && !done && !skip_done && (P.k > k2_max_k() || (P.tune.k2_big_min_k > 0 && P.k >= (uint32_t)P.tune.k2_big_min_k))) {
        launch_k2_topk_big(L, P, prev, cand_off, ncand, cand, out.idx, out.val, out.cnt, out.stride, s);
        return;
    }
    if (k2_wave_path(P)) {
        const uint32_t ns = ((rank_limit ? std::min(P.cand_stride, std::max(1u, limited_cands)) : P.cand_stride) + 63u) / 64u;
        const dim3 grid((P.nrows + 3u) / 4u), block(256);
        if (ns <= 1) hipLaunchKernelGGL(k2_topk_wave<1>, grid, block, 0, s, a);
        else if (ns <= 2) hipLaunchKernelGGL(k2_topk_wave<2>, grid, block, 0, s, a);
        else if (ns <= 4) hipLaunchKernelGGL(k2_topk_wave<4>, grid, block, 0, s, a);
        else if (ns <= 8) hipLaunchKernelGGL(k2_topk_wave<8>, grid, block, 0, s, a);
        else if (ns <= 13) hipLaunchKernelGGL(k2_topk_wave<13>, grid, block, 0, s, a);
        else if (ns <= 16) hipLaunchKernelGGL(k2_topk_wave<16>, grid, block, 0, s, a);
        else if (ns <= 24) hipLaunchKernelGGL(k2_topk_wave<24>, grid, block, 0, s, a);
        else hipLaunchKernelGGL(k2_topk_wave<32>, grid, block, 0, s, a);
    } else if (P.k <= 64) {
        hipLaunchKernelGGL(k2_topk_reg, dim3(P.nrows), dim3(64), 0, s, a);
    } else {
        const size_t lds = (size_t)P.k * 8;
        if (P.k > k2_max_k()) fail("k2: only_topk/beam_size " + std::to_string(P.k) + " exceeds the device limit " + std::to_string(k2_max_k()));
        if (lds > 48 * 1024)
            XRL_HIP(hipFuncSetAttribute(reinterpret_cast<const void*>(&k2_topk_lds), hipFuncAttributeMaxDynamicSharedMemorySize, (int)lds));
        hipLaunchKernelGGL(k2_topk_lds, dim3(P.nrows), dim3(64), lds, s, a);
    }
    XRL_LAUNCH_CHECK();
}

}
```

pecos_amd/csrc/xrl_kernels.h:

```cpp
#pragma once
#include "xrl_model.h"

namespace xrl {

struct QueriesDev {
    const uint64_t* row_ptr;
    const uint32_t* col_idx;
    const float* val;
    uint32_t rows, cols;
    int dense;
    uint64_t nnz;
};

struct BeamDev {
    uint32_t* idx;
    float* val;
    uint32_t* cnt;
    uint32_t stride;
};

struct K1Tune { int wpb = 1, lds_pad = 0, ablate = 0, k1g_variant = 0, pres_mode = 1, tile_rows = 1, k2_big_min_k = 0; };

struct LayerPlan {
    uint32_t row0, nrows;
    uint32_t beam_in;
    uint32_t k;
    uint32_t cand_stride;
    PostProc pp;
    int first_layer;
    int implicit_root;
    int prune;
    int bias_first;
    int layer;
    K1Tune tune;
    uint32_t* fb_host = nullptr;
    uint32_t* fb_dev = nullptr;
};

void launch_k0_prolongate(const LayerDev& L, const LayerPlan& P, const QueriesDev& X, BeamDev prev, uint32_t* cand_off,
                          uint32_t* ncand, void* items, hipStream_t s, uint32_t item_ranks = 0xFFFFFFFFu );
void launch_k0b_remaining(const LayerDev& L, const LayerPlan& P, const QueriesDev& X, BeamDev prev, const uint32_t* cand_off, const uint32_t* done,
                          uint32_t first_rank, void* items, uint32_t* n_items, hipStream_t s, uint32_t end_rank = 0xFFFFFFFFu);
bool k2_wave_path(const LayerPlan& P);
size_t k0_item_bytes();
void launch_k1(const LayerDev& L, const LayerPlan& P, const QueriesDev& X, const void* items, const uint32_t* n_items,
               float* cand, int group, hipStream_t s);
void launch_sort_items(const LayerDev& L, uint64_t n_slots, const void* items, void* sorted, uint32_t* H,
                       uint32_t* start, hipStream_t s,
                       const uint32_t* n_dev = nullptr);
void launch_sort_queries(BeamDev prev, uint32_t nrows, uint32_t n_keys, uint32_t* H, uint32_t* start, uint32_t* perm, hipStream_t s);
uint32_t qsort_max_keys();
size_t qsort_hist_bytes(uint32_t nrows, uint32_t n_keys);
void launch_step_marker(hipStream_t s);
uint32_t sort_max_tiles();
size_t sort_hist_bytes(uint64_t n_slots, uint32_t n_tiles);
void launch_k2_topk(const LayerDev& L, const LayerPlan& P, BeamDev prev, const uint32_t* cand_off,
                    const uint32_t* ncand, const float* cand, BeamDev out, hipStream_t s,
                    uint32_t rank_limit = 0 , uint32_t limited_cands = 0 ,
                    uint32_t* done = nullptr , const uint32_t* skip_done = nullptr ,
                    const uint32_t* xok = nullptr );
constexpr int kStatsPerLayer = 8;
void launch_stats(const LayerDev& L, const LayerPlan& P, const QueriesDev& X, BeamDev prev, const uint32_t* ncand, const void* items,
                  double* out8, hipStream_t s, uint64_t item_slots = 0 );
void launch_k3_inner_products(const uint64_t* x_ptr, const uint32_t* x_idx, const float* x_val, int x_dense,
                              const uint64_t* w_ptr, const uint32_t* w_idx, const float* w_val, int w_dense,
                              uint32_t dim, uint64_t len, const uint32_t* rows, const uint32_t* cols,
                              float* out, hipStream_t s);

unsigned long long* k1_phase_buffer();
void k1_phase_read(unsigned long long out[8], bool reset);
void launch_k4_selected(const uint64_t* col_ptr, const uint32_t* row_idx, const float* val, uint32_t w_rows, float bias,
                        const QueriesDev& X, const uint32_t* pair_q, const uint32_t* node, const uint32_t* ppos,
                        const uint64_t* prev_off, const float* prev_val, float* out_val, uint64_t n_pairs,
                        const PostProc& pp, int first_layer, hipStream_t s);
uint32_t k1g_cols(const LayerDev& L);
void launch_k1g(const LayerDev& L, const LayerPlan& P, const QueriesDev& X, const void* items_sorted, const uint32_t* start,
                uint32_t* blk_start, const uint32_t* x_ok, float* cand, hipStream_t s);
void launch_xguard(const QueriesDev& X, uint32_t row0, uint32_t nrows, float wmax, uint32_t* ok, hipStream_t s);
void launch_k1c_csc(const LayerDev& L, const uint64_t* col_ptr, const uint32_t* row_idx, const float* val, const LayerPlan& P,
                    const QueriesDev& X, BeamDev prev, const uint32_t* cand_off, const uint32_t* ncand, float* cand, hipStream_t s);
void launch_concat_csr(const uint64_t* in_ptr, const uint32_t* in_idx, const float* in_val, const float* emb, uint32_t rows,
                       uint32_t sparse_cols, uint32_t dense_cols, int normalize_emb, uint64_t* out_ptr, uint32_t* out_idx, float* out_val, hipStream_t s);
void launch_tfidf_weight(const uint64_t* row_ptr, const uint32_t* col_idx, const float* count, const float* idf, uint32_t rows, uint32_t cols,
                         int binary, int sublinear_tf, int norm_p, float* out, hipStream_t s,
                         uint32_t seg_stride = 1, uint32_t seg_off = 0, uint32_t* err = nullptr);
int k1_auto_group(const LayerDev& L, const Layer& host, int dense);
bool k1t_serves(const LayerDev& L, const QueriesDev& X);
struct K1TSelect { BeamDev prev; const uint32_t* xok; BeamDev out; uint32_t* done; uint32_t* cand_off; uint32_t* ncand; };
bool k1t_selects(const LayerDev& L, const LayerPlan& P, const QueriesDev& X);
void launch_k1t(const LayerDev& L, const LayerPlan& P, const QueriesDev& X, const void* items, const uint32_t* n_items, float* cand, hipStream_t s,
                const K1TSelect* sel = nullptr);
uint32_t k1q_regs(const LayerDev& L, uint32_t beam_in, uint32_t k, bool dense_x);
void launch_k1q(const LayerDev* const* Ls, const LayerPlan* Ps, int n, const QueriesDev& X, BeamDev prev, BeamDev out,
                hipStream_t s, float prune_wmax, uint32_t* out_xok = nullptr,
                const uint32_t* qperm = nullptr );
size_t k2_max_k();
void launch_k2_topk_big(const LayerDev& L, const LayerPlan& P, BeamDev prev, const uint32_t* cand_off, const uint32_t* ncand, const float* cand,
                        uint32_t* out_idx, float* out_val, uint32_t* out_cnt, uint32_t out_stride, hipStream_t s);

constexpr int kEnsembleMaxModels = 8;
constexpr uint32_t kEnsembleMaxTotal = 1024;
enum { kEnsembleAverage = 0, kEnsembleFinish = 1, kEnsembleRankAverage = 2 };
struct EnsembleArgs {
    const uint32_t* idx[kEnsembleMaxModels];
    const float* val[kEnsembleMaxModels];
    const uint32_t* cnt[kEnsembleMaxModels];
    uint32_t stride[kEnsembleMaxModels];
    uint32_t n_models, rows;
    int mode;
    int has_threshold;
    float threshold;
    uint32_t only_topk;
    uint32_t* out_idx;
    float* out_val;
    uint32_t* out_cnt;
    uint32_t out_stride;
};
uint32_t ensemble_slots(uint32_t stride_sum);
void launch_ensemble(const EnsembleArgs& A, uint32_t* mm_scratch, hipStream_t s);

constexpr uint32_t kSelectMaxStride = 1024;
constexpr uint32_t kSelectNone = 0xFFFFFFFFu;
enum { kSelectOk = 0, kSelectOutOfRange = 1, kSelectTwice = 2, kSelectNoParent = 3 };
struct SelectTreeLayer {
    const uint32_t* parent;
    const uint32_t* crank;
    uint32_t c_rows, pad;
};
struct SelectPlanArgs {
    const uint32_t* sel_idx; const uint32_t* sel_cnt;
    uint32_t sel_stride;
    uint32_t row0, nrows;
    uint32_t depth, nr_labels;
    const SelectTreeLayer* tree;
    uint32_t* node; uint32_t* ppos; uint32_t* cnt; uint64_t layer_elems, layer_rows;
    uint32_t* out_idx; uint32_t* out_cnt; uint32_t out_stride;
    unsigned long long* status;
};
void launch_select_plan(const SelectPlanArgs& A, hipStream_t s);
struct SelectScoreArgs {
    const uint64_t* col_ptr; const uint32_t* row_idx; const float* val; uint32_t w_rows; float bias;
    const uint32_t* node; uint32_t node_stride;
    const uint32_t* ppos; const uint32_t* cnt;
    const float* prev_val;
    float* out_val; uint32_t out_stride;
    uint32_t row0, nrows, sel_stride;
};
void launch_k4_selected_dev(const SelectScoreArgs& A, const QueriesDev& X, const PostProc& pp, hipStream_t s);

}
```

pecos_amd/csrc/xrl_model.h:

```cpp
#pragma once
#include <memory>
#include <mutex>
#include <string>
#include <vector>

#include "xrl_common.h"
#include "xrl_feedback.h"
#include "xrl_io.h"

namespace xrl {

constexpr uint32_t kMaxTileCols = 128;
constexpr uint32_t kNoBias = 0xFFFFFFFFu;
constexpr uint32_t kMissing = 0x80000000u;

enum PPKind : int { PP_NOOP = 0, PP_SIGMOID = 1, PP_LOG_SIGMOID = 2, PP_LP_HINGE = 3, PP_LOG_LP_HINGE = 4 };
struct PostProc { int kind = PP_NOOP; int p = 0; };
PostProc parse_post_processor(const char* name);

struct TileDesc {
    uint32_t col_begin;
    uint32_t ncols;
    uint32_t nrows;
    uint32_t bias_slot;
    uint64_t rowptr_base;
    uint64_t ent_base;
};

struct Entry { uint32_t col; float val; };
struct BmWord { uint32_t bits; uint32_t rank; };
struct alignas(16) BmWord64 { uint32_t lo, hi, rank, ext0; };
inline uint32_t pack_row_extent(uint32_t start, uint32_t len) { return start | ((len - 1u) << 25); }

struct LayerDev {
    const TileDesc* tiles;
    const uint32_t* ptile;
    const uint32_t* chunk_col;
    const BmWord* bitmap;
    const BmWord64* bitmap64;
    uint32_t nwords64;
    const uint32_t* bucket;
    uint32_t bk_shift, bk_n, bk_levels;
    const uint32_t* row_ext;
    const uint32_t* row_idx;
    const Entry* entries;
    const uint32_t* perm_inv;
    const float* chunk_alg_bytes;
    const float* bias_prod;
    uint32_t n_parents, n_children, n_tiles, nwords, w_rows;
    uint32_t max_tiles_per_parent, max_tile_cols;
    float bias;
    int has_bias;
    const uint32_t* wd;
    uint64_t d_ld;
    uint32_t d_gp_log2;
    uint32_t d_max_tiles;
    const uint32_t* d_ptile;
    const uint32_t* d_tcol;
    int d_sparse_ok;
    const uint32_t* pres;
    uint32_t pres_words;
    int d_full;
    const uint32_t* tile_parent;
    const uint32_t* wd01; uint32_t wd01_c1;
    const float* wt; const uint64_t* wt_base; uint32_t wt_stride; uint64_t wt_bytes;
    int d_regular;
};

struct ConstraintView {
    bool active = false;
    DevBuf d_chunk_col, d_perm_inv;
    std::vector<uint32_t> chunk_sizes_desc;
    uint64_t kept = 0;
    uint64_t cand_bound(uint32_t beam) const;
    void clear() { active = false; d_chunk_col.release(); d_perm_inv.release(); chunk_sizes_desc.clear(); kept = 0; }
};

struct Layer {
    uint32_t w_rows = 0, w_cols = 0, c_rows = 0, c_cols = 0;
    float bias = 0.f;
    float w_absmax = 0.f;
    uint32_t only_topk = 0;
    PostProc pp;
    std::string pp_name;
    bool reordered = false;
    uint32_t n_children = 0;
    uint32_t n_tiles = 0, nwords = 0, max_tiles_per_parent = 0, max_tile_cols = 0, max_chunk_cols = 0;
    uint64_t nnz = 0, total_rows = 0;
    std::vector<uint32_t> chunk_sizes_desc;
    std::vector<uint64_t> h_c_ptr; std::vector<uint32_t> h_c_idx, h_parent;
    std::string w_path; std::shared_ptr<HostCsc> w_host;
    DevBuf d_csc_ptr, d_csc_idx, d_csc_val; bool csc_ready = false;
    DevBuf d_sel_parent, d_sel_crank;
    DevBuf d_tiles, d_ptile, d_chunk_col, d_bitmap, d_row_ptr, d_row_idx, d_entries, d_perm_inv, d_chunk_alg, d_bias_prod;
    DevBuf d_bucket, d_bitmap64;
    DevBuf d_wd, d_dptile, d_dtcol, d_tile_parent, d_pres;
    DevBuf d_wt, d_wt_base;
    uint64_t dense_bytes = 0;
    uint32_t bk_shift = 0, bk_n = 0, bk_levels = 0;
    ConstraintView view;
    LayerDev dev{};
    uint64_t device_bytes = 0;
    uint64_t buffer_bytes() const;
    uint64_t cand_bound(uint32_t beam) const;
    uint64_t cand_bound_kept(uint32_t beam) const { return view.active ? view.cand_bound(beam) : cand_bound(beam); }
};

struct ProfileSlot { std::string name; uint32_t layer; uint32_t launches = 0; double ms = 0; };
struct PendingEvent { hipEvent_t a, b; size_t slot; };

struct LaneWs {
    DevBuf beam_idx[2], beam_val[2], beam_cnt[2];
    DevBuf cand_off, ncand, cand;
    DevBuf items, items_sorted, sort_hist, sort_start;
    DevBuf blk_start, x_ok;
    DevBuf qperm, qsort_hist, qsort_start;
    DevBuf prune_done, prune_cnt;
};
struct Workspace {
    LaneWs lane[2];
    DevBuf stats;
    DevBuf x_ptr, x_idx, x_val;
    DevBuf out_idx, out_val, out_cnt;
    PinnedBuf h_idx, h_val, h_cnt;
    PinnedBuf stage[3];
    PinnedBuf stage_ptr;
    DevBuf init_idx, init_val, init_cnt;
    DevBuf sel_node, sel_ppos, sel_cnt, sel_val[2], sel_status;
};

struct Model {
    int device = 0;
    int weight_matrix_type = 2;
    std::vector<std::unique_ptr<Layer>> layers;
    uint32_t nr_features = 0, nr_labels = 0, nr_codes = 0;
    hipStream_t stream = nullptr;
    hipStream_t aux_stream = nullptr;
    hipEvent_t ws_done = nullptr;
    hipStream_t ws_stream = nullptr;
    hipStream_t copy_stream = nullptr;
    hipStream_t d2h_stream = nullptr;
    std::vector<hipEvent_t> d2h_events;
    std::vector<hipEvent_t> events;
    struct HostLanes { hipEvent_t done[2] = {nullptr, nullptr}; hipStream_t strm[2] = {nullptr, nullptr}; hipEvent_t join = nullptr; } host_lanes;
    std::mutex mu;
    std::unique_ptr<Workspace> ws;
    bool constrained = false;
    bool csc_route = false;
    DevBuf d_wd01;
    DevBuf d_sel_tree; bool sel_tree_ready = false;
    PruneFeedback fb;
    struct Options {
        int k1_group = 0;
        int k1_wpb = 1, k1_lds_pad = 0, k1_ablate = 0;
        int k1g_variant = 0;
        int64_t max_batch_rows = 0;
        int overlap_min_rows = 0;
        int prune = 1;
        int k2_big_min_k = 0;
        int tile_rows = 1;
        int dense_layers = 1;
        int k1q_fuse = 3;
        int k1g_first = 0;
        int k1g_min_items = 16;
        int adaptive = 1;
        int presence = 1;
        int leaf_fuse = 1;
        int prune_mid = 1;
        int sort_rest = 1;
        int sort_rest_min = 32768;
        int qsort = 1;
        int qsort_min_parents = 64, qsort_min_rows = 131072;
        int sort_min_tiles = 0;
        int host_register = 0;
        int host_batch_mb = 12;
        int host_pipeline = 1;
    } opt;
    std::string src_path; int src_kind = -1;
    std::vector<std::unique_ptr<Model>> replicas;
    bool profiling = false;
    std::vector<ProfileSlot> profile;
    std::vector<PendingEvent> pending;
    Model();
    ~Model();
    uint64_t device_bytes() const;
};

uint32_t split_chunk(const uint64_t* cum, uint32_t n, uint64_t limit);
uint64_t layout_tile_rows(const uint32_t* rptr, uint32_t nrows, bool align, uint32_t* ext);

std::unique_ptr<Layer> compile_layer(const HostCsc& W, const HostCsc& C, float bias, uint32_t only_topk,
                                     const std::string& post_processor,
                                     const std::vector<uint32_t>* perm_inv_override = nullptr, uint32_t orig_rows = 0,
                                     bool structure_only = false);
std::unique_ptr<Model> load_model_from_disk(const std::string& path, int weight_matrix_type);
void finalize_model(Model& m);
std::unique_ptr<Model> load_mmap_model_from_disk(const std::string& path);
void compile_mmap_model(const std::string& npz_path, const std::string& mmap_path);
void ensure_device_csc(Layer& L);
void set_output_constraint(Model& m, const uint32_t* labels, uint64_t n, bool on_device, hipStream_t s, const char* what);
void clear_output_constraint(Model& m);
void ensure_device_tree(Model& m);
void k1t_shape(uint32_t max_tile_cols, int& g, int& nr);
void launch_tile_rows(const LayerDev& L, uint64_t total_floats, uint32_t* wt, hipStream_t s);
inline bool k1q_merged01_addressable(uint32_t w_rows) { return ((uint64_t)w_rows + 2) * 256ull < 0xFFFFFFF0ull; }
void launch_merge01(const uint32_t* wd0, uint64_t ld0, uint32_t k0, const uint32_t* wd1, uint64_t ld1, uint32_t c1, uint32_t rows, uint32_t* out, hipStream_t s);
void launch_presence(const uint32_t* wd, uint64_t ld, uint32_t rows, uint32_t gp_log2, uint32_t n_tiles, uint32_t pres_words, uint32_t* pres, hipStream_t s);
void launch_densify(const uint64_t* col_ptr, const uint32_t* row_idx, const float* val, const uint32_t* src_col,
                    const uint32_t* dst_off, uint32_t n_children, uint32_t w_rows, uint64_t ld, uint32_t* wd, hipStream_t s);

}
```

pecos_amd/csrc/xrl_predict.cpp:

```cpp
#include "xrl_predict.h"
#include "xrl_constrain.h"

#include <algorithm>
#include <cstdio>
#include <cstdlib>

namespace xrl {

size_t profile_slot(Model& m, const char* name, uint32_t layer) {
    for (size_t i = 0; i < m.profile.size(); ++i)
        if (m.profile[i].layer == layer && m.profile[i].name == name) return i;
    m.profile.push_back(ProfileSlot{name, layer});
    return m.profile.size() - 1;
}

namespace {

uint32_t k1g_first_slots(const Layer& L, uint32_t beam_in, int forced = 0) {
    if (forced > 0) return (uint32_t)std::max<int64_t>(1, std::min<int64_t>(beam_in > 1 ? (int64_t)beam_in - 1 : 1, forced));
    return (uint32_t)std::max<uint64_t>(1, std::min<uint64_t>(beam_in > 1 ? beam_in - 1 : 1, 64 / std::max<uint64_t>(1, L.cand_bound(1))));
}

struct LayerShape { uint32_t k, beam_in, cand_stride; PostProc pp; };

enum RouteKind { ROUTE_CSC, ROUTE_K1G, ROUTE_K1Q, ROUTE_TILE, ROUTE_CONSTRAINED };
struct Route {
    RouteKind kind;
    size_t last;
    bool sorted_last;
    int mode;
    int group;
    bool pruned;
    uint32_t J;
    uint32_t stage_end[3]; int n_stage;
    bool fuse, fuse_k0;
    bool sorts_rest;
};

struct Batch {
    Model& m; const Model::Options& opt; const QueriesDev& X; const PredictOpts& o; const std::vector<LayerShape>& shape;
    BeamDev result{}; uint32_t beam_stride = 1;
    bool has_init = false, csc = false, stats = false; double* stats_dev = nullptr;
    uint64_t nb = 1; int lanes = 1;
    PruneFeedback::Plan fb{};
    float prune_wmax = 0.0f;
    hipEvent_t k1_done = nullptr; size_t ev_next = 0;
    uint64_t row0 = 0; uint32_t nrows = 0; hipStream_t S = nullptr;
    bool x_ok_done = false;
    BeamDev beam[2]{};
    uint32_t *cand_off, *ncand, *sort_hist, *sort_start, *blk_start, *x_ok, *qperm, *qsort_hist, *qsort_start, *prune_done, *prune_cnt;
    float* cand; void *items, *items_sorted;

    void begin_batch(const LaneWs& lw, hipStream_t s, uint64_t r0, uint32_t n) {
        auto u32 = [](const DevBuf& d) { return d.as<uint32_t>(); };
        row0 = r0; nrows = n; S = s; x_ok_done = false;
        for (int i = 0; i < 2; ++i) beam[i] = BeamDev{u32(lw.beam_idx[i]), lw.beam_val[i].as<float>(), u32(lw.beam_cnt[i]), beam_stride};
        cand_off = u32(lw.cand_off); ncand = u32(lw.ncand); cand = lw.cand.as<float>(); items = lw.items.p; items_sorted = lw.items_sorted.p;
        sort_hist = u32(lw.sort_hist); sort_start = u32(lw.sort_start); blk_start = u32(lw.blk_start); x_ok = u32(lw.x_ok);
        qperm = u32(lw.qperm); qsort_hist = u32(lw.qsort_hist); qsort_start = u32(lw.qsort_start); prune_done = u32(lw.prune_done); prune_cnt = u32(lw.prune_cnt);
    }
    bool unstaged(size_t l) const { return l < (size_t)kFbLayers && fb.unstaged[l]; }
    LayerPlan make_plan(size_t l) const {
        LayerPlan P{};
        P.layer = (int)l; P.row0 = (uint32_t)row0; P.nrows = nrows;
        P.beam_in = shape[l].beam_in; P.k = shape[l].k; P.cand_stride = shape[l].cand_stride; P.pp = shape[l].pp;
        P.tune = K1Tune{opt.k1_wpb, opt.k1_lds_pad, opt.k1_ablate, opt.k1g_variant, opt.presence, opt.tile_rows, opt.k2_big_min_k};
        P.first_layer = (l == 0 && (!has_init || o.no_prev_pred)) ? 1 : 0; P.implicit_root = (l == 0 && !has_init) ? 1 : 0;
        P.bias_first = (m.weight_matrix_type == 1 && !X.dense) ? 1 : 0; P.prune = (opt.prune && !unstaged(l)) ? 1 : 0;
        if (opt.prune && opt.adaptive && !stats && l < (size_t)kFbLayers) { P.fb_host = m.fb.host; P.fb_dev = m.fb.dev.as<uint32_t>(); }
        return P;
    }
    BeamDev beam_prev(size_t l) const {
        if (l > 0 || !has_init) return l > 0 ? beam[(l - 1) & 1] : BeamDev{};
        const BeamDev& i = *o.initial;
        return BeamDev{i.idx + row0 * i.stride, i.val + row0 * i.stride, i.cnt + row0, i.stride};
    }
    BeamDev beam_out(size_t l) const {
        if (l + 1 < shape.size()) return beam[l & 1];
        return BeamDev{result.idx + row0 * result.stride, result.val + row0 * result.stride, result.cnt + row0, result.stride};
    }
    hipEvent_t next_event() {
        if (ev_next == m.events.size()) { hipEvent_t e; XRL_HIP(hipEventCreateWithFlags(&e, hipEventDisableTiming)); m.events.push_back(e); }
        return m.events[ev_next++];
    }
    void chain(hipStream_t from, hipStream_t to) { hipEvent_t e = next_event(); XRL_HIP(hipEventRecord(e, from)); XRL_HIP(hipStreamWaitEvent(to, e, 0)); }
    static bool debug_sync() { static const bool on = [] { const char* e = std::getenv("XRL_DEBUG_SYNC"); return e && e[0] == '1'; }(); return on; }
    bool named() const { return m.profiling || debug_sync(); }
    template <class F> void timed(const char* name, uint32_t layer, F&& fn) {
        if (debug_sync()) {
            std::fprintf(stderr, "[xrl debug] %s layer %u rows %llu+%u\n", name, layer, (unsigned long long)row0, nrows); std::fflush(stderr);
            fn(); const hipError_t e = hipStreamSynchronize(S);
            if (e != hipSuccess) fail(std::string("device fault in ") + name + " (layer " + std::to_string(layer) + ", rows " + std::to_string(row0) + "+" + std::to_string(nrows) + "): " + hipGetErrorString(e));
            return;
        }
        profiled(m, S, name, layer, fn);
    }
    void need_x_ok() {
        if (!x_ok_done) timed("xguard", 0, [&] { launch_xguard(X, (uint32_t)row0, nrows, prune_wmax, x_ok, S); });
        x_ok_done = true;
    }
};

std::vector<LayerShape> resolve_layers(const Model& m, const QueriesDev& X, const PredictOpts& o) {
    if (!X.dense && X.cols != m.nr_features && X.cols != m.layers[0]->w_rows)
        fail("X.shape[1] (" + std::to_string(X.cols) + ") != nr_features (" + std::to_string(m.nr_features) + ")");
    if (X.dense && X.cols < m.nr_features)
        fail("dense X has fewer columns (" + std::to_string(X.cols) + ") than nr_features (" + std::to_string(m.nr_features) + ")");
    const size_t T = m.layers.size();
    const bool has_init = o.initial != nullptr;
    std::vector<LayerShape> shape(T);
    for (size_t l = 0; l < T; ++l) {
        const Layer& L = *m.layers[l]; LayerShape& s = shape[l];
        const uint32_t ov = (l == T - 1) ? o.only_topk : o.beam_size;
        s.k = ov ? ov : L.only_topk;
        if (s.k == 0) fail("layer " + std::to_string(l) + ": only_topk resolved to 0");
        s.pp = o.post_processor ? parse_post_processor(o.post_processor) : L.pp;
        uint64_t bin = (l == 0) ? (has_init ? std::max<uint32_t>(1, o.initial_max) : 1) : std::min<uint64_t>(shape[l - 1].k, shape[l - 1].cand_stride);
        if (!(l == 0 && has_init)) bin = std::min<uint64_t>(bin, L.c_cols ? L.c_cols : 1);
        s.beam_in = (uint32_t)std::max<uint64_t>(1, bin);
        const uint64_t cb = std::max<uint64_t>(1, (l == 0 && has_init && o.initial_cand_bound) ? o.initial_cand_bound : L.cand_bound_kept(s.beam_in));
        if (cb > 0x7FFFFFFFull) fail("candidate row too long; lower beam_size");
        s.cand_stride = (uint32_t)cb;
    }
    return shape;
}

void size_batches(Batch& b, uint64_t n_rows) {
    uint32_t cs_max = 1;
    for (const LayerShape& s : b.shape) cs_max = std::max(cs_max, s.cand_stride);
    uint64_t nb = std::min<uint64_t>(std::max<uint64_t>(1, kCandBudgetBytes / ((uint64_t)cs_max * 4)), 1u << 22);
    if (b.opt.max_batch_rows > 0) nb = std::min<uint64_t>(nb, (uint64_t)b.opt.max_batch_rows);
    nb = std::min<uint64_t>(nb, std::max<uint64_t>(1, std::max<uint64_t>(n_rows, b.o.reserve_rows)));
    b.lanes = (b.opt.overlap_min_rows > 0 && !b.stats && !b.m.profiling && n_rows >= (uint64_t)b.opt.overlap_min_rows) ? 2 : 1;
    b.nb = b.lanes == 2 ? std::min<uint64_t>(nb, (n_rows + 1) / 2) : nb;
}

int tile_mode(const Batch& b, size_t l, uint64_t rows) {
    const Layer& L = *b.m.layers[l];
    if (L.n_tiles > sort_max_tiles()) return 0;
    const uint64_t slots = rows * b.shape[l].beam_in * L.max_tiles_per_parent;
    if (b.X.dense && b.opt.dense_layers && b.opt.k1g_min_items > 0 && !b.csc && k1g_cols(L.dev) != 0 && b.shape[l].k <= k2_max_k() &&
        slots / std::max<uint32_t>(1, L.n_tiles) >= (uint64_t)b.opt.k1g_min_items) return 3;
    return (b.opt.sort_min_tiles > 0 && L.n_tiles >= (uint32_t)b.opt.sort_min_tiles) ? 1 : 0;
}

Route route_layer(const Batch& b, size_t l, uint64_t nrows) {
    const Model& m = b.m; const Model::Options& opt = b.opt; const Layer& L = *m.layers[l];
    const uint32_t beam_in = b.shape[l].beam_in;
    Route r{}; r.last = l; r.J = 1;
    if (m.constrained) { r.kind = ROUTE_CONSTRAINED; return r; }
    r.mode = tile_mode(b, l, nrows);
    r.sorts_rest = opt.sort_rest != 0 && !b.stats && L.n_tiles <= sort_max_tiles() && L.n_tiles >= 64u;
    if (b.csc) { r.kind = ROUTE_CSC; return r; }
    const LayerPlan P = b.make_plan(l);
    const bool boundable = !P.implicit_root && !P.first_layer && P.pp.kind != PP_NOOP && beam_in > 1 && k2_wave_path(P);
    if (!b.stats && r.mode == 3) {
        r.kind = ROUTE_K1G; r.pruned = opt.prune && boundable;
        r.J = r.pruned ? k1g_first_slots(L, beam_in, opt.k1g_first) : beam_in;
        return r;
    }
    const bool dense_x = b.X.dense != 0 || opt.dense_layers >= 2;
    auto regs = [&](size_t ll) { return k1q_regs(m.layers[ll]->dev, b.shape[ll].beam_in, b.shape[ll].k, dense_x); };
    auto runs_k1q = [&](size_t ll) { return opt.dense_layers && !b.stats && tile_mode(b, ll, nrows) != 3 && regs(ll) != 0; };
    if (runs_k1q(l)) {
        r.kind = ROUTE_K1Q;
        auto narrow = [&](size_t ll) { return regs(ll) <= (uint32_t)std::min(3, opt.k1q_fuse); };
        while (opt.k1q_fuse && narrow(l) && r.last + 1 < b.shape.size() && r.last + 1 - l < 8 && runs_k1q(r.last + 1) && narrow(r.last + 1)) ++r.last;
        const uint32_t nk = m.layers[r.last]->dev.n_parents;
        r.sorted_last = opt.qsort != 0 && !b.X.dense && r.last > 0 && nrows >= (uint64_t)std::max(1, opt.qsort_min_rows) &&
                        nk >= (uint32_t)std::max(2, opt.qsort_min_parents) && nk <= qsort_max_keys();
        return r;
    }
    r.kind = ROUTE_TILE; r.group = opt.k1_group > 0 ? opt.k1_group : k1_auto_group(L.dev, L, b.X.dense);
    if (b.unstaged(l) && r.mode == 0 && r.sorts_rest) r.mode = 1;
    r.pruned = opt.prune && !b.unstaged(l) && boundable;
    if (b.stats) {
        if (r.mode == 3) r.J = k1g_first_slots(L, beam_in, opt.k1g_first);
        else if (opt.dense_layers && regs(l) != 0) {
            if (regs(l) <= 1) r.pruned = false;
            else r.J = std::max<uint32_t>(1, (64u >> L.dev.d_gp_log2) / std::max<uint32_t>(1, L.dev.d_max_tiles));
        }
        if (r.J >= beam_in) r.pruned = false;
    } else if (r.mode != 0) r.pruned = false;
    if (!r.pruned) return r;
    r.stage_end[r.n_stage++] = r.J;
    if (opt.prune_mid != 0 && beam_in >= 16u && !b.stats) r.stage_end[r.n_stage++] = std::min<uint32_t>(beam_in - 1u, r.J + 4u);
    r.stage_end[r.n_stage++] = beam_in;
    r.fuse = opt.leaf_fuse != 0 && r.J == 1 && !b.stats && k1t_selects(L.dev, P, b.X);
    r.fuse_k0 = r.fuse && opt.leaf_fuse != 2 && beam_in <= 32u;
    return r;
}

void reserve_scratch(const Batch& b, Workspace& ws, uint64_t n_rows) {
    const Model& m = b.m; const size_t T = b.shape.size(); const uint64_t nb = b.nb;
    uint32_t bin_max = 1, cs_max = 1; uint64_t slots_max = 1;
    for (size_t l = 0; l < T; ++l) {
        bin_max = std::max(bin_max, b.shape[l].beam_in); cs_max = std::max(cs_max, b.shape[l].cand_stride); slots_max = std::max<uint64_t>(slots_max, nb * b.shape[l].beam_in * m.layers[l]->max_tiles_per_parent);
    }
    size_t sorted = 0, hist = 0, starts = 0, x_ok = 0, done = 0, cnt = 0, qperm = 0, qhist = 0, qstarts = 0;
    for (const uint64_t rows : {nb, n_rows % nb}) {
        for (size_t l = 0; l < T && rows; ++l) {
            const Route r = route_layer(b, l, rows); const Layer& L = *m.layers[l];
            const bool staged_tile = r.kind == ROUTE_TILE && r.pruned;
            if (r.mode != 0 || (b.opt.prune && r.sorts_rest)) { hist = std::max(hist, sort_hist_bytes(nb * b.shape[l].beam_in * L.max_tiles_per_parent, L.n_tiles)); starts = std::max(starts, ((size_t)L.n_tiles + 1) * 4); }
            if (starts || staged_tile) sorted = slots_max * k0_item_bytes();
            if (staged_tile || (r.kind == ROUTE_K1G && r.pruned)) { done = (size_t)nb * 4; cnt = 256; }
            if (r.kind == ROUTE_K1G || staged_tile || (r.kind == ROUTE_K1Q && b.opt.prune && r.last + 1 < T)) x_ok = (size_t)nb * 4;
            const uint32_t nk = m.layers[r.last]->dev.n_parents;
            if (r.kind == ROUTE_K1Q && r.sorted_last) { qperm = (size_t)nb * 4; qhist = std::max(qhist, qsort_hist_bytes((uint32_t)nb, nk)); qstarts = std::max(qstarts, ((size_t)nk + 1) * 4); }
        }
    }
    for (int ln = 0; ln < b.lanes; ++ln) {
        LaneWs& lw = ws.lane[ln];
        for (int i = 0; i < 2; ++i) { lw.beam_idx[i].reserve(nb * b.beam_stride * 4); lw.beam_val[i].reserve(nb * b.beam_stride * 4); lw.beam_cnt[i].reserve(nb * 4); }
        lw.items.reserve(slots_max * k0_item_bytes());
        lw.cand_off.reserve(nb * bin_max * 4); lw.ncand.reserve(nb * 4); lw.cand.reserve(nb * (uint64_t)cs_max * 4);
        lw.items_sorted.reserve(sorted); lw.sort_hist.reserve(hist); lw.sort_start.reserve(starts); lw.blk_start.reserve(starts);
        lw.x_ok.reserve(x_ok); lw.prune_done.reserve(done); lw.prune_cnt.reserve(cnt);
        lw.qperm.reserve(qperm); lw.qsort_hist.reserve(qhist); lw.qsort_start.reserve(qstarts);
    }
    if (b.stats) m.ws->stats.reserve(T * kStatsPerLayer * sizeof(double));
}

void launch_csc_layer(Batch& b, size_t l) {
    Layer& L = *b.m.layers[l]; const LayerPlan P = b.make_plan(l); const BeamDev prev = b.beam_prev(l);
    ensure_device_csc(L);
    b.timed("k0_prolongate", l, [&] { launch_k0_prolongate(L.dev, P, b.X, prev, b.cand_off, b.ncand, b.items, b.S); });
    b.timed("k1c_csc", l, [&] { launch_k1c_csc(L.dev, L.d_csc_ptr.as<uint64_t>(), L.d_csc_idx.as<uint32_t>(), L.d_csc_val.as<float>(), P, b.X, prev, b.cand_off, b.ncand, b.cand, b.S); });
    b.timed("k2_topk", l, [&] { launch_k2_topk(L.dev, P, prev, b.cand_off, b.ncand, b.cand, b.beam_out(l), b.S); });
}

void launch_constrained_layer(Batch& b, size_t l) {
    Layer& L = *b.m.layers[l]; LayerPlan P = b.make_plan(l); const BeamDev prev = b.beam_prev(l);
    P.fb_host = nullptr; P.fb_dev = nullptr; P.prune = 0;
    LayerDev V = L.dev;
    if (L.view.active) { V.chunk_col = L.view.d_chunk_col.as<uint32_t>(); V.perm_inv = L.view.d_perm_inv.as<uint32_t>(); }
    const int chain = (b.csc || b.X.dense) ? kChainCsc : kChainChunked;
    b.timed("k0_constrained", l, [&] { launch_k0_prolongate(V, P, b.X, prev, b.cand_off, b.ncand, b.items, b.S, 0); });
    b.timed("k1p_constrained", l, [&] { launch_k1p_constrained(V, L.d_csc_ptr.as<uint64_t>(), L.d_csc_idx.as<uint32_t>(), L.d_csc_val.as<float>(), P, chain, b.X, prev, b.cand_off, b.ncand, b.cand, b.S); });
    b.timed("k2_constrained", l, [&] { launch_k2_topk(V, P, prev, b.cand_off, b.ncand, b.cand, b.beam_out(l), b.S); });
}

void launch_k1g_layer(Batch& b, size_t l, const Route& r) {
    const Layer& L = *b.m.layers[l]; const QueriesDev& X = b.X; hipStream_t S = b.S;
    const LayerPlan P = b.make_plan(l); const BeamDev prev = b.beam_prev(l), out = b.beam_out(l);
    const uint32_t J = r.J, rest = P.beam_in - J;
    b.need_x_ok();
    LayerPlan PA = P; PA.beam_in = J;
    b.timed("k0_prolongate", l, [&] { launch_k0_prolongate(L.dev, P, X, prev, b.cand_off, b.ncand, b.items, S, J); });
    b.timed("k1_sort_items", l, [&] { launch_sort_items(L.dev, (uint64_t)b.nrows * J * L.max_tiles_per_parent, b.items, b.items_sorted, b.sort_hist, b.sort_start, S); });
    b.timed("k1g_dense_x", l, [&] { launch_k1g(L.dev, PA, X, b.items_sorted, b.sort_start, b.blk_start, b.x_ok, b.cand, S); });
    if (!r.pruned) { b.timed("k2_topk", l, [&] { launch_k2_topk(L.dev, P, prev, b.cand_off, b.ncand, b.cand, out, S); }); return; }
    LayerPlan PB = P; PB.beam_in = rest;
    b.timed("k2_topk", l, [&] { launch_k2_topk(L.dev, P, prev, b.cand_off, b.ncand, b.cand, out, S, J, (uint32_t)L.cand_bound(J), b.prune_done, nullptr, b.x_ok); });
    b.timed("k0b_remaining", l, [&] { launch_k0b_remaining(L.dev, P, X, prev, b.cand_off, b.prune_done, J, b.items, b.prune_cnt, S); });
    b.timed("k1_sort_items_rest", l, [&] { launch_sort_items(L.dev, (uint64_t)b.nrows * rest * L.max_tiles_per_parent, b.items, b.items_sorted, b.sort_hist, b.sort_start, S, b.prune_cnt); });
    b.timed("k1g_dense_x_rest", l, [&] { launch_k1g(L.dev, PB, X, b.items_sorted, b.sort_start, b.blk_start, b.x_ok, b.cand, S); });
    b.timed("k2_topk_rest", l, [&] { launch_k2_topk(L.dev, P, prev, b.cand_off, b.ncand, b.cand, out, S, 0, 0, nullptr, b.prune_done); });
}

void launch_k1q_group(Batch& b, size_t l, const Route& r) {
    const QueriesDev& X = b.X; hipStream_t S = b.S; const LayerDev* Ls[8]; LayerPlan Ps[8];
    for (size_t ll = l; ll <= r.last; ++ll) {
        Ls[ll - l] = &b.m.layers[ll]->dev; Ps[ll - l] = b.make_plan(ll);
        Ps[ll - l].fb_host = Ps[0].fb_host; Ps[ll - l].fb_dev = Ps[0].fb_dev;
    }
    const BeamDev prev = b.beam_prev(l);
    const size_t n_shared = r.last - l + (r.sorted_last ? 0 : 1), ls = r.last;
    const char* const single = X.dense ? "k1q_dense_x" : "k1q_dense";
    char fused[48] = "";
    if (n_shared > 1 && b.named()) std::snprintf(fused, sizeof fused, "k1q_fused_%s%zu_%zu", X.dense ? "x_" : "", l, l + n_shared - 1);
    uint32_t* xok_out = nullptr;
    if (!b.x_ok_done && b.opt.prune && r.last + 1 < b.shape.size()) { xok_out = b.x_ok; b.x_ok_done = true; }
    BeamDev pv = prev;
    if (n_shared) {
        pv = b.beam_out(l + n_shared - 1);
        b.timed(n_shared > 1 ? fused : single, l, [&] { launch_k1q(Ls, Ps, (int)n_shared, X, prev, pv, S, b.prune_wmax, xok_out); });
        xok_out = nullptr;
    }
    if (!r.sorted_last) return;
    b.timed("k1_sort_queries", ls, [&] { launch_sort_queries(pv, b.nrows, Ls[ls - l]->n_parents, b.qsort_hist, b.qsort_start, b.qperm, S); });
    b.timed(single, ls, [&] { launch_k1q(Ls + (ls - l), Ps + (ls - l), 1, X, pv, b.beam_out(ls), S, b.prune_wmax, xok_out, b.qperm); });
}

const char* const kK1Name[2][3] = {{"k1_sparse", "k1_sparse_mid", "k1_sparse_rest"}, {"k1_dense", "k1_dense_mid", "k1_dense_rest"}};

void launch_tile_layer(Batch& b, size_t l, const Route& r) {
    Model& m = b.m; const Layer& L = *m.layers[l]; const QueriesDev& X = b.X; hipStream_t S = b.S;
    const LayerPlan P = b.make_plan(l); const BeamDev prev = b.beam_prev(l), out = b.beam_out(l);
    const uint32_t beam_in = P.beam_in, nrows = b.nrows, J = r.J;
    const char* const* k1_name = kK1Name[X.dense ? 1 : 0];
    double* const stats = b.stats ? b.stats_dev + kStatsPerLayer * l : nullptr;
    if (!r.pruned) {
        b.timed("k0_prolongate", l, [&] { launch_k0_prolongate(L.dev, P, X, prev, b.cand_off, b.ncand, b.items, S); });
        if (r.mode != 0) b.timed("k1_sort_items", l, [&] { launch_sort_items(L.dev, (uint64_t)nrows * beam_in * L.max_tiles_per_parent, b.items, b.items_sorted, b.sort_hist, b.sort_start, S); });
        if (b.lanes == 2 && b.k1_done) XRL_HIP(hipStreamWaitEvent(S, b.k1_done, 0));
        LayerPlan PU = P; PU.fb_host = nullptr;
        b.timed(k1_name[0], l, [&] { launch_k1(L.dev, PU, X, r.mode == 1 ? b.items_sorted : b.items, r.mode == 1 ? b.sort_start + L.n_tiles : nullptr, b.cand, r.group, S); });
        if (b.lanes == 2) { b.k1_done = b.next_event(); XRL_HIP(hipEventRecord(b.k1_done, S)); }
        b.timed("k2_topk", l, [&] { launch_k2_topk(L.dev, P, prev, b.cand_off, b.ncand, b.cand, out, S); });
        if (stats) launch_stats(L.dev, P, X, prev, b.ncand, b.items, stats, S);
        return;
    }
    const uint64_t slots_b = (uint64_t)nrows * (beam_in - J) * L.max_tiles_per_parent;
    b.need_x_ok();
    if (!r.fuse_k0) b.timed("k0_prolongate", l, [&] { launch_k0_prolongate(L.dev, P, X, prev, b.cand_off, b.ncand, b.items, S, J); });
    if (b.lanes == 2 && b.k1_done) XRL_HIP(hipStreamWaitEvent(S, b.k1_done, 0));
    if (r.fuse) {
        const K1TSelect sel{prev, b.x_ok, out, b.prune_done, b.cand_off, b.ncand};
        b.timed("k1_sparse", l, [&] { launch_k1t(L.dev, P, X, r.fuse_k0 ? nullptr : b.items, nullptr, b.cand, S, &sel); });
    } else {
        LayerPlan PA = P; PA.beam_in = J;
        b.timed(k1_name[0], l, [&] { launch_k1(L.dev, PA, X, b.items, nullptr, b.cand, r.group, S); });
        b.timed("k2_topk", l, [&] { launch_k2_topk(L.dev, P, prev, b.cand_off, b.ncand, b.cand, out, S, J, (uint32_t)L.cand_bound(J), b.prune_done, nullptr, b.x_ok); });
    }
    if (stats) XRL_HIP(hipMemsetAsync(b.items_sorted, 0xFF, slots_b * k0_item_bytes(), S));
    bool srt = r.sorts_rest;
    if (srt && P.fb_host && b.opt.sort_rest_min > 0) {
        const uint32_t seen = m.fb.word(fb_items_word((int)l));
        const uint64_t need = std::max<uint64_t>((uint64_t)b.opt.sort_rest_min, 32ull * L.n_tiles);
        if (seen != kFbPending && (uint64_t)seen < need) srt = false;
    }
    if (P.fb_host) m.fb.tile_slots[l] = (uint64_t)nrows * (beam_in - r.stage_end[r.n_stage - 2]) * L.max_tiles_per_parent;
    for (int st = 1; st < r.n_stage; ++st) {
        const uint32_t r0 = r.stage_end[st - 1], r1 = r.stage_end[st]; const bool last = st == r.n_stage - 1;
        LayerPlan PB = P; PB.beam_in = r1 - r0; PB.tune.wpb = 4;
        b.timed(last ? "k0b_remaining" : "k0b_remaining_mid", l, [&] { launch_k0b_remaining(L.dev, P, X, prev, b.cand_off, b.prune_done, r0, srt ? b.items : b.items_sorted, b.prune_cnt, S, r1); });
        if (srt) b.timed(last ? "k1_sort_items_rest" : "k1_sort_items_mid", l, [&] { launch_sort_items(L.dev, (uint64_t)nrows * (r1 - r0) * L.max_tiles_per_parent, b.items, b.items_sorted, b.sort_hist, b.sort_start, S, b.prune_cnt); });
        b.timed(k1_name[last ? 2 : 1], l, [&] { launch_k1(L.dev, PB, X, b.items_sorted, srt ? b.sort_start + L.n_tiles : b.prune_cnt, b.cand, r.group, S); });
        if (b.lanes == 2 && last) { b.k1_done = b.next_event(); XRL_HIP(hipEventRecord(b.k1_done, S)); }
        if (last) b.timed("k2_topk_rest", l, [&] { launch_k2_topk(L.dev, P, prev, b.cand_off, b.ncand, b.cand, out, S, 0, 0, nullptr, b.prune_done); });
        else b.timed("k2_topk_mid", l, [&] { launch_k2_topk(L.dev, P, prev, b.cand_off, b.ncand, b.cand, out, S, r1, (uint32_t)L.cand_bound(r1), b.prune_done, b.prune_done, b.x_ok); });
        if (stats && last) { launch_stats(L.dev, P, X, prev, b.ncand, b.items, stats, S, (uint64_t)nrows * J * L.max_tiles_per_parent); launch_stats(L.dev, PB, X, prev, nullptr, b.items_sorted, stats, S, slots_b); }
    }
}

void launch_batch(Batch& b) {
    for (size_t l = 0; l < b.shape.size(); ++l) {
        const Route r = route_layer(b, l, b.nrows);
        switch (r.kind) {
            case ROUTE_CSC: launch_csc_layer(b, l); break;
            case ROUTE_K1G: launch_k1g_layer(b, l, r); break;
            case ROUTE_K1Q: launch_k1q_group(b, l, r); break;
            case ROUTE_TILE: launch_tile_layer(b, l, r); break;
            case ROUTE_CONSTRAINED: launch_constrained_layer(b, l); break;
        }
        l = r.last;
    }
}
}

PruneFeedback::Plan PruneFeedback::begin_predict(size_t n_layers, bool sample) {
    Plan plan;
    if (!host) {
        XRL_HIP(hipHostMalloc(reinterpret_cast<void**>(&host), kFbHostWords * 4, hipHostMallocDefault));
        for (int i = 0; i < kFbHostWords; ++i) host[i] = i < kFbCounterWords ? 0u : kFbPending;
        dev.reserve(kFbCounterWords * 4); XRL_HIP(hipMemset(dev.p, 0, kFbCounterWords * 4));
    }
    for (int l = 0; l < (int)std::min<size_t>(n_layers, kFbLayers); ++l) {
        if (sample && unstaged[l]) {
            bool decided = false, stage_again = false;
            if (probing[l]) {
                const uint32_t sn = word(fb_seen_word(l)), sec = word(fb_second_word(l)), dseen = sn - seen[l], dsec = sec - second[l];
                const uint32_t cnt = word(fb_items_word(l));
                if (dseen >= kMinSamples) { decided = true; stage_again = !((double)dsec > kSecondShare * (double)dseen); seen[l] = sn; second[l] = sec; }
                else if (cnt != kFbPending && tile_slots[l] > 0) { decided = true; stage_again = !((double)cnt > kItemShare * (double)tile_slots[l]); }
                if (decided) { probing[l] = 0; unstaged_calls[l] = 0; if (stage_again) unstaged[l] = 0; }
            }
            if (unstaged[l] && ++unstaged_calls[l] >= kReprobe) {
                unstaged_calls[l] = 0; probing[l] = 1; plan.probed[l] = true;
                if (!decided) { seen[l] = word(fb_seen_word(l)); second[l] = word(fb_second_word(l)); }
                host[fb_items_word(l)] = kFbPending; tile_slots[l] = 0;
            }
        } else if (sample) {
            const uint32_t sn = word(fb_seen_word(l)), sec = word(fb_second_word(l)), dseen = sn - seen[l], dsec = sec - second[l];
            if (dseen >= kMinSamples) {
                if ((double)dsec > kSecondShare * (double)dseen) { unstaged[l] = 1; unstaged_calls[l] = 0; probing[l] = 0; }
                seen[l] = sn; second[l] = sec;
            }
            const uint32_t cnt = word(fb_items_word(l));
            if (cnt != kFbPending && tile_slots[l] > 0 && (double)cnt > kItemShare * (double)tile_slots[l]) { unstaged[l] = 1; unstaged_calls[l] = 0; probing[l] = 0; }
        }
        plan.unstaged[l] = unstaged[l] != 0 && !plan.probed[l];
    }
    return plan;
}

uint32_t effective_topk(const Model& m, uint32_t only_topk) { return only_topk ? only_topk : m.layers.back()->only_topk; }

void predict_device(Model& m, const QueriesDev& X, const PredictOpts& o, uint32_t* d_out_idx, float* d_out_val,
                    uint32_t* d_out_cnt, uint32_t out_stride, hipStream_t stream, bool sync, uint32_t row_begin, uint32_t row_count) {
    const size_t T = m.layers.size();
    if (row_begin > X.rows) fail("predict: row range outside X");
    const uint64_t row_end = std::min<uint64_t>(X.rows, (uint64_t)row_begin + row_count), n_rows = row_end - row_begin;
    if (!m.ws) m.ws = std::make_unique<Workspace>();
    if (!stream) stream = m.stream;
    if (m.ws_done && m.ws_stream != stream) XRL_HIP(hipStreamWaitEvent(stream, m.ws_done, 0));
    static const bool step_marker = [] { const char* e = std::getenv("XRL_STEP_MARKER"); return e && e[0] == '1'; }();
    if (step_marker && !o.stats_out) launch_step_marker(stream);

    const std::vector<LayerShape> shape = resolve_layers(m, X, o);
    if (shape[T - 1].k > out_stride) fail("out_stride smaller than the effective only_topk");
    Batch b{m, m.opt, X, o, shape, BeamDev{d_out_idx, d_out_val, d_out_cnt, out_stride}};
    b.has_init = o.initial != nullptr; b.csc = o.csc_route || m.csc_route; b.stats = o.stats_out != nullptr;
    for (size_t l = 0; l < T; ++l) {
        if (l + 1 < T) b.beam_stride = std::max(b.beam_stride, shape[l].k);
        b.prune_wmax = std::max(b.prune_wmax, m.layers[l]->w_absmax);
    }
    if (!(b.prune_wmax <= 3.0e38f)) b.prune_wmax = INFINITY;
    size_batches(b, n_rows);
    if (m.opt.prune && m.opt.adaptive && !m.constrained) b.fb = m.fb.begin_predict(T, !b.stats);
    reserve_scratch(b, *m.ws, n_rows);
    if (b.stats) { b.stats_dev = m.ws->stats.as<double>(); XRL_HIP(hipMemsetAsync(m.ws->stats.p, 0, T * kStatsPerLayer * sizeof(double), stream)); }

    hipStream_t lane_stream[2] = {stream, stream};
    if (b.lanes == 2) {
        if (!m.aux_stream) XRL_HIP(hipStreamCreateWithFlags(&m.aux_stream, hipStreamNonBlocking));
        lane_stream[1] = m.aux_stream;
        b.chain(stream, m.aux_stream);
    }

    uint64_t batch = 0;
    for (uint64_t row0 = row_begin; row0 < row_end; row0 += b.nb, ++batch) {
        const int ln = (int)(batch % (uint64_t)b.lanes);
        b.begin_batch(m.ws->lane[ln], lane_stream[ln], row0, (uint32_t)std::min<uint64_t>(b.nb, row_end - row0));
        launch_batch(b);
    }
    if (b.lanes == 2) b.chain(m.aux_stream, stream);

    if (!m.ws_done) XRL_HIP(hipEventCreateWithFlags(&m.ws_done, hipEventDisableTiming));
    XRL_HIP(hipEventRecord(m.ws_done, stream)); m.ws_stream = stream;

    if (o.stats_out || sync) XRL_HIP(hipStreamSynchronize(stream));
    if (o.stats_out) XRL_HIP(hipMemcpy(o.stats_out, m.ws->stats.p, T * kStatsPerLayer * sizeof(double), hipMemcpyDeviceToHost));
}

void resolve_profile(Model& m) {
    if (m.pending.empty()) return;
    XRL_HIP(hipSetDevice(m.device));
    XRL_HIP(hipDeviceSynchronize());
    for (auto& ev : m.pending) {
        float ms = 0.f;
        XRL_HIP(hipEventElapsedTime(&ms, ev.a, ev.b));
        m.profile[ev.slot].ms += ms;
        m.profile[ev.slot].launches += 1;
        (void)hipEventDestroy(ev.a); (void)hipEventDestroy(ev.b);
    }
    m.pending.clear();
}

}
```

Before: 97.81 million queries/s.

## Compact unfinished queries into a list for the tail stage of tiled layers

The first-stage top-k (fused k1t or k2) now appends each query that is not yet done to a compact list. The remaining-rank item builder, the persistent k1 list kernel and the rest top-k then walk only that list instead of scanning every row and checking the done flag. A grid-stride persistent k1 variant is used when feedback shows few remaining items. This cuts wasted wave launches on finished queries, at the cost of atomics, an extra buffer and a new leaf_tail option.

```diff
diff --git a/pecos_amd/csrc/xrl_abi.cpp b/pecos_amd/csrc/xrl_abi.cpp
--- a/pecos_amd/csrc/xrl_abi.cpp
+++ b/pecos_amd/csrc/xrl_abi.cpp
@@ -503,7 +503,7 @@
 
 #define XRL_OPT(name) {#name, &Model::Options::name}
 static const struct { const char* name; int Model::Options::*field; } kIntOptions[] = {
-    XRL_OPT(k1_group), XRL_OPT(sort_min_tiles), XRL_OPT(sort_rest), XRL_OPT(sort_rest_min), XRL_OPT(prune_mid), XRL_OPT(leaf_fuse), XRL_OPT(tile_rows),
+    XRL_OPT(k1_group), XRL_OPT(sort_min_tiles), XRL_OPT(sort_rest), XRL_OPT(sort_rest_min), XRL_OPT(prune_mid), XRL_OPT(leaf_fuse), XRL_OPT(leaf_tail), XRL_OPT(tile_rows),
     XRL_OPT(k2_big_min_k), XRL_OPT(qsort), XRL_OPT(qsort_min_parents), XRL_OPT(qsort_min_rows), XRL_OPT(presence), XRL_OPT(adaptive), XRL_OPT(prune),
     XRL_OPT(host_pipeline), XRL_OPT(host_batch_mb), XRL_OPT(host_register), XRL_OPT(overlap_min_rows),
     XRL_OPT(dense_layers), XRL_OPT(k1q_fuse), XRL_OPT(k1g_first), XRL_OPT(k1g_min_items), XRL_OPT(k1g_variant),
diff --git a/pecos_amd/csrc/xrl_k0.hip b/pecos_amd/csrc/xrl_k0.hip
--- a/pecos_amd/csrc/xrl_k0.hip
+++ b/pecos_amd/csrc/xrl_k0.hip
@@ -80,9 +80,58 @@
     }
 }
 
+__global__ void __launch_bounds__(256)
+k0b_remaining_list(const uint32_t* __restrict__ chunk_col, const uint32_t* __restrict__ ptile, const TileDesc* __restrict__ tiles,
+                   uint32_t nrows, uint32_t beam_in, uint32_t first_rank, uint32_t end_rank, uint32_t cand_stride, const uint32_t* __restrict__ p_idx,
+                   const float* __restrict__ p_val, const uint32_t* __restrict__ p_cnt, uint32_t p_stride, const uint32_t* __restrict__ cand_off,
+                   const uint32_t* __restrict__ rest_q, const uint32_t* __restrict__ rest_cnt, uint32_t lpq, ItemDesc* __restrict__ items,
+                   uint32_t* __restrict__ n_items, const uint64_t* __restrict__ x_row_ptr) {
+    const uint32_t lane = threadIdx.x & 63u;
+    const uint32_t wave0 = blockIdx.x * 4u + (threadIdx.x >> 6), n_waves = gridDim.x * 4u;
+    const uint32_t nq = min(*rest_cnt, nrows);
+    const uint32_t qpw = 64u / lpq, qi = lane / lpq, j0 = first_rank + lane % lpq;
+    for (uint32_t g = wave0; g * qpw < nq; g += n_waves) {
+        const uint32_t i = g * qpw + qi;
+        uint32_t q = (qi < qpw && i < nq) ? rest_q[i] : nrows;
+        const bool live = q < nrows;
+        if (!live) q = 0;
+        const uint32_t cnt = live ? min(min(p_cnt[q], beam_in), end_rank) : 0u;
+        uint32_t n = 0;
+        for (uint32_t j = j0; j < cnt; j += lpq) { const uint32_t parent = p_idx[(size_t)q * p_stride + j]; n += ptile[parent + 1] - ptile[parent]; }
+        uint32_t incl = n;
+#pragma unroll
+        for (int d = 1; d < 64; d <<= 1) { const uint32_t y = (uint32_t)__shfl_up((int)incl, d, 64); if (lane >= (uint32_t)d) incl += y; }
+        const uint32_t total = (uint32_t)__shfl((int)incl, 63, 64);
+        if (total == 0) continue;
+        uint32_t base = 0;
+        if (lane == 63u) base = atomicAdd(n_items, total);
+        base = (uint32_t)__shfl((int)base, 63, 64) + incl - n;
+        uint64_t xb = 0; uint32_t xl = 0;
+        if (n != 0 && x_row_ptr) { xb = x_row_ptr[q]; xl = (uint32_t)(x_row_ptr[q + 1] - xb); }
+        for (uint32_t j = j0; n != 0 && j < cnt; j += lpq) {
+            const uint32_t parent = p_idx[(size_t)q * p_stride + j];
+            const float ps = p_val[(size_t)q * p_stride + j];
+            const uint32_t cb = chunk_col[parent], t0 = ptile[parent], nt = ptile[parent + 1] - t0;
+            const uint32_t off = cand_off[(size_t)q * beam_in + j];
+            for (uint32_t tt = 0; tt < nt; ++tt)
+                items[base++] = make_item(q, t0 + tt, q * cand_stride + off + (tiles[t0 + tt].col_begin - cb), ps, xb, xl);
+        }
+    }
+}
+
 void launch_k0b_remaining(const LayerDev& L, const LayerPlan& P, const QueriesDev& X, BeamDev prev, const uint32_t* cand_off, const uint32_t* done,
-                          uint32_t first_rank, void* items, uint32_t* n_items, hipStream_t s, uint32_t end_rank) {
+                          uint32_t first_rank, void* items, uint32_t* n_items, hipStream_t s, uint32_t end_rank, const uint32_t* rest_q, const uint32_t* rest_cnt) {
     if (P.nrows == 0) return;
+    if (rest_q) {
+        if (!rest_cnt) fail("k0b: the list of unfinished queries needs its count");
+        const uint32_t hi = std::min(P.beam_in, end_rank);
+        const uint32_t lpq = std::max(1u, std::min(hi > first_rank ? hi - first_rank : 1u, 64u));
+        hipLaunchKernelGGL(k0b_remaining_list, dim3(std::min<uint32_t>((P.nrows + 3u) / 4u, 512u)), dim3(256), 0, s, L.chunk_col, L.ptile, L.tiles, P.nrows, P.beam_in,
+                           first_rank, end_rank, P.cand_stride, prev.idx, prev.val, prev.cnt, prev.stride, cand_off, rest_q, rest_cnt, lpq, static_cast<ItemDesc*>(items),
+                           n_items, X.dense ? nullptr : X.row_ptr + P.row0);
+        XRL_LAUNCH_CHECK();
+        return;
+    }
     XRL_HIP(hipMemsetAsync(n_items, 0, 4, s));
     hipLaunchKernelGGL(k0b_remaining, dim3((P.nrows + 255) / 256), dim3(256), 0, s, L.chunk_col, L.ptile, L.tiles, P.nrows, P.beam_in, first_rank, end_rank,
                        P.cand_stride, prev.idx, prev.val, prev.cnt, prev.stride, cand_off, done, static_cast<ItemDesc*>(items), n_items,
diff --git a/pecos_amd/csrc/xrl_k1.hip b/pecos_amd/csrc/xrl_k1.hip
--- a/pecos_amd/csrc/xrl_k1.hip
+++ b/pecos_amd/csrc/xrl_k1.hip
@@ -21,6 +21,7 @@
     uint32_t n_vblocks;
     unsigned long long* phase;
     uint32_t* fb_out;
+    uint32_t stride_vblocks;
 };
 
 template <int G, int PPC, class ACC>
@@ -69,14 +70,14 @@
 #ifndef XRL_K1_WPE
 #define XRL_K1_WPE 5
 #endif
-template <int G, int NS, int PPC, bool DENSE, int LK>
-__global__ void __launch_bounds__(256) __attribute__((amdgpu_waves_per_eu(XRL_K1_WPE, 8))) k1_kernel(K1Args a) {
+template <int G, int NS, int PPC, bool DENSE, int LK, bool PERSIST>
+__device__ __forceinline__ void k1_run(const K1Args& a) {
     constexpr int W = K1Cfg<G, NS>::W, H = K1Cfg<G, NS>::H, UH = K1Cfg<G, NS>::UH, P = K1Cfg<G, NS>::P, U = K1Cfg<G, NS>::U,
                   NB = K1Cfg<G, NS>::NB, TAIL = K1Cfg<G, NS>::TAIL;
     extern __shared__ __attribute__((aligned(16))) unsigned char smem_all[];
     const uint32_t wave = threadIdx.x >> 6;
-    const uint32_t vblock = blockIdx.x * (blockDim.x >> 6) + wave;
-    if (vblock >= a.n_vblocks) return;
+    const uint32_t vblock0 = blockIdx.x * (blockDim.x >> 6) + wave;
+    if (vblock0 >= a.n_vblocks) return;
     unsigned char* smem = smem_all + (size_t)wave * a.lds_per_wave;
     uint2* uq = reinterpret_cast<uint2*>(smem);
     uint2* hq = reinterpret_cast<uint2*>(uq + W * (UH + TAIL));
@@ -92,6 +93,7 @@
 #else
     auto tick = [](int) {};
 #endif
+    auto body = [&](const uint32_t vblock) {
     ItemDesc it;
     if (!fetch_item<W>(a.items, a.n_items, a.n_slots, a.fb_out, vblock, grp, lane, it)) return;
     const bool active = it.tile != kNoTile;
@@ -267,10 +269,22 @@
         if (lane == 0) { for (int i = 0; i < 5; ++i) atomicAdd(&a.phase[i], t_ph[i]); atomicAdd(&a.phase[5], 1ull); }
     }
 #endif
-}
+    };
+    if constexpr (PERSIST) {
+        const uint32_t nb = (*a.n_items + W - 1) / W;
+        if (a.fb_out && vblock0 == 0 && lane == 0) *a.fb_out = *a.n_items;
+        for (uint32_t vb = vblock0; vb < nb; vb += a.stride_vblocks) { body(vb); wave_sync_lds(); }
+    } else body(vblock0);
+}
+
+template <int G, int NS, int PPC, bool DENSE, int LK>
+__global__ void __launch_bounds__(256) __attribute__((amdgpu_waves_per_eu(XRL_K1_WPE, 8))) k1_kernel(K1Args a) { k1_run<G, NS, PPC, DENSE, LK, false>(a); }
+
+template <int G, int NS, int PPC, int LK>
+__global__ void __launch_bounds__(256) __attribute__((amdgpu_waves_per_eu(4, 8))) k1_list_kernel(K1Args a) { k1_run<G, NS, PPC, false, LK, true>(a); }
 
 template <class KERNEL>
-static void launch_k1_any(KERNEL kernel, K1Args a, int W, size_t lds_wave, const K1Tune& tune, hipStream_t s) {
+static void launch_k1_any(KERNEL kernel, K1Args a, int W, size_t lds_wave, const K1Tune& tune, hipStream_t s, uint32_t list_grid = 0) {
     lds_wave = (lds_wave + (size_t)std::max(0, tune.lds_pad) + 15) & ~(size_t)15;
     int wpb = (tune.wpb == 2 || tune.wpb == 4) ? tune.wpb : 1;
     while (wpb > 1 && lds_wave * wpb > 160 * 1024) wpb >>= 1;
@@ -282,7 +296,13 @@
     const uint64_t blocks = (vblocks + wpb - 1) / wpb;
     if (vblocks > 0x7FFFFFFFull) fail("k1: grid too large; lower max_batch_rows");
     a.lds_per_wave = (uint32_t)lds_wave; a.n_vblocks = (uint32_t)vblocks;
-    hipLaunchKernelGGL(kernel, dim3((uint32_t)blocks), dim3(64 * wpb), lds, s, a);
+    uint64_t grid = blocks;
+    a.stride_vblocks = 0;
+    if (list_grid) {
+        grid = std::min<uint64_t>(blocks, ((uint64_t)list_grid + 7) & ~7ull);
+        a.stride_vblocks = (uint32_t)(grid * wpb); a.n_vblocks = (uint32_t)std::min<uint64_t>(vblocks, grid * wpb);
+    }
+    hipLaunchKernelGGL(kernel, dim3((uint32_t)grid), dim3(64 * wpb), lds, s, a);
     XRL_LAUNCH_CHECK();
 }
 
@@ -304,10 +324,10 @@
     return 32;
 }
 
-void launch_k1(const LayerDev& L, const LayerPlan& P, const QueriesDev& X, const void* items, const uint32_t* n_items,
-               float* cand, int group, hipStream_t s) {
-    if (P.nrows == 0) return;
-    if ((P.tune.tile_rows >= 2 || (P.tune.tile_rows == 1 && !n_items)) && P.tune.ablate == 0 && k1t_serves(L, X)) { launch_k1t(L, P, X, items, n_items, cand, s); return; }
+bool launch_k1(const LayerDev& L, const LayerPlan& P, const QueriesDev& X, const void* items, const uint32_t* n_items,
+               float* cand, int group, hipStream_t s, uint32_t list_grid) {
+    if (P.nrows == 0) return false;
+    if ((P.tune.tile_rows >= 2 || (P.tune.tile_rows == 1 && !n_items)) && P.tune.ablate == 0 && k1t_serves(L, X)) { launch_k1t(L, P, X, items, n_items, cand, s); return false; }
     K1Args a;
     a.L = L; a.X = X; a.items = static_cast<const ItemDesc*>(items); a.n_items = n_items; a.cand = cand;
     a.n_slots = (uint64_t)P.nrows * P.beam_in * L.max_tiles_per_parent;
@@ -318,13 +338,23 @@
     a.phase = ((ablate & 64) && ((ablate >> 8) == 0 || (ablate >> 8) == P.layer + 1)) ? k1_phase_buffer() : nullptr;
     a.fb_out = (n_items && P.fb_host && P.layer >= 0 && P.layer < kFbLayers) ? P.fb_host + fb_items_word(P.layer) : nullptr;
     const int ppc = pp_class(P.pp);
+    const bool persist = n_items != nullptr && list_grid > 0 && ablate == 0 && !X.dense && ppc == 0;
+    bool ran_list = false;
 #define XRL_K1_PP(GG, NN, DD, LL) do { if (ppc) launch_k1_any(&k1_kernel<GG, NN, 1, DD, LL>, a, 64 / GG, lds, P.tune, s); else launch_k1_any(&k1_kernel<GG, NN, 0, DD, LL>, a, 64 / GG, lds, P.tune, s); } while (0)
+#define XRL_K1_LIST(GG, NN, LL) launch_k1_any(&k1_list_kernel<GG, NN, 0, LL>, a, 64 / GG, lds, P.tune, s, list_grid)
 #define XRL_K1(GG, NN) do { \
         const size_t lds = K1Cfg<GG, NN>::lds_bytes(a.acc_stride); \
         if (X.dense) XRL_K1_PP(GG, NN, true, 0); \
         else if (L.bucket) XRL_K1_PP(GG, NN, false, 1); \
         else if (L.bitmap64) XRL_K1_PP(GG, NN, false, 2); \
         else XRL_K1_PP(GG, NN, false, 0); } while (0)
+#define XRL_K1P(GG, NN) do { \
+        if (!persist) { XRL_K1(GG, NN); break; } \
+        const size_t lds = K1Cfg<GG, NN>::lds_bytes(a.acc_stride); \
+        ran_list = true; \
+        if (L.bucket) XRL_K1_LIST(GG, NN, 1); \
+        else if (L.bitmap64) XRL_K1_LIST(GG, NN, 2); \
+        else XRL_K1_LIST(GG, NN, 0); } while (0)
     if (group < 1 || group > 64 || (group & (group - 1))) fail("k1: lanes-per-item must be a power of two in [1, 64]");
     auto max_ns = [](int g) { return g < 8 ? 1u : (g == 32 ? 4u : 2u); };
     auto units = [&](int g) { return (L.max_tile_cols + (uint32_t)g - 1) / (uint32_t)g; };
@@ -335,12 +365,15 @@
     case 2: XRL_K1(2, 1); break;
     case 4: XRL_K1(4, 1); break;
     case 8: if (ns <= 1) XRL_K1(8, 1); else XRL_K1(8, 2); break;
-    case 16: if (ns <= 1) XRL_K1(16, 1); else XRL_K1(16, 2); break;
-    case 32: if (ns <= 1) XRL_K1(32, 1); else if (ns == 2) XRL_K1(32, 2); else if (ns == 3) XRL_K1(32, 3); else XRL_K1(32, 4); break;
+    case 16: if (ns <= 1) XRL_K1P(16, 1); else XRL_K1P(16, 2); break;
+    case 32: if (ns <= 1) XRL_K1P(32, 1); else if (ns == 2) XRL_K1P(32, 2); else if (ns == 3) XRL_K1P(32, 3); else XRL_K1P(32, 4); break;
     default: if (ns <= 1) XRL_K1(64, 1); else XRL_K1(64, 2); break;
     }
+#undef XRL_K1P
 #undef XRL_K1
+#undef XRL_K1_LIST
 #undef XRL_K1_PP
-}
-
-}
+    return ran_list;
+}
+
+}
diff --git a/pecos_amd/csrc/xrl_k1t.hip b/pecos_amd/csrc/xrl_k1t.hip
--- a/pecos_amd/csrc/xrl_k1t.hip
+++ b/pecos_amd/csrc/xrl_k1t.hip
@@ -29,6 +29,7 @@
     int mult;
     const uint32_t* p_idx; const uint64_t* x_row_ptr;
     uint32_t cand_stride; uint32_t* cand_off; uint32_t* ncand;
+    uint32_t* rest_q; uint32_t* rest_cnt;
 };
 
 template <int NR> struct RowVec;
@@ -202,6 +203,15 @@
             const uint32_t total = (uint32_t)__shfl((int)incl, 31, 32);
             if (mine) a.cand_off[q * a.beam_in + (uint32_t)lig] = incl - wd;
             if (qv && !d && lig == 0) a.ncand[q] = total;
+        }
+        if (a.rest_q) {
+            const unsigned long long um = __ballot(qv && !d && lig == 0);
+            if (um) {
+                uint32_t base = 0;
+                if (lane_e == 0) base = atomicAdd(a.rest_cnt, (uint32_t)__popcll(um));
+                base = (uint32_t)__shfl((int)base, 0, 64);
+                if (qv && !d && lig == 0) a.rest_q[base + (grp ? (uint32_t)(um & 1ull) : 0u)] = (uint32_t)q;
+            }
         }
         if (active && !d) {
             float* __restrict__ out = a.cand + it.out_off;
@@ -307,6 +317,8 @@
             if ((uint64_t)P.nrows * P.cand_stride > 0xFFFFFFFFull) fail("k1t: candidate buffer exceeds 2^32 floats; lower max_batch_rows");
             a.p_idx = sel->prev.idx; a.x_row_ptr = X.row_ptr + P.row0; a.cand_stride = P.cand_stride; a.cand_off = sel->cand_off; a.ncand = sel->ncand;
         }
+        if (sel->rest_q && !sel->rest_cnt) fail("k1t: the list of unfinished queries needs its count");
+        a.rest_q = sel->rest_q; a.rest_cnt = sel->rest_cnt;
     }
     const dim3 grid((a.n_vblocks + 3u) / 4u), block(256);
 #define XRL_K1T_L(GG, NN, BB, SS) do { \
diff --git a/pecos_amd/csrc/xrl_k2.hip b/pecos_amd/csrc/xrl_k2.hip
--- a/pecos_amd/csrc/xrl_k2.hip
+++ b/pecos_amd/csrc/xrl_k2.hip
@@ -1,4 +1,6 @@
 #include <hip/hip_runtime.h>
+
+#include <type_traits>
 
 #include "xrl_device.h"
 #include "xrl_kernels.h"
@@ -19,6 +21,7 @@
     uint32_t* done;
     const uint32_t* skip_done;
     const uint32_t* xok;
+    uint32_t* rest_q; uint32_t* rest_cnt;
 };
 
 __device__ __forceinline__ uint32_t k2_child_id(const K2Args& a, uint64_t q, uint32_t pos) {
@@ -128,14 +131,7 @@
 }
 
 template <int NS>
-__global__ void __launch_bounds__(256) k2_topk_wave(K2Args a) {
-    __shared__ uint2 sc_all[4 * 64];
-    const int lane = threadIdx.x & 63;
-    const uint32_t wave = __builtin_amdgcn_readfirstlane(threadIdx.x >> 6);
-    const uint32_t q32 = blockIdx.x * 4u + wave;
-    if (q32 >= a.nrows) return;
-    const uint64_t q = q32;
-    if (a.skip_done && a.skip_done[q]) return;
+__device__ __forceinline__ void k2_wave_query(const K2Args& a, const uint64_t q, uint2* sc, const int lane) {
     uint32_t n = min(a.ncand[q], (uint32_t)(64 * NS));
     const uint32_t bcnt0 = a.implicit_root ? 1u : min(a.p_cnt[q], a.beam_in);
     const uint32_t rl = min(a.rank_limit, a.beam_in - 1u);
@@ -160,10 +156,13 @@
     if (a.done) {
         bool d = true;
         if (limited) d = a.xok[q] != 0u && ps_next == ps_next && wave_count_ge<NS>(key, score_key(a.mult ? fmaxf(ps_next, 0.0f) : ps_next)) >= a.k;
-        if (lane == 0) a.done[q] = d ? 1u : 0u;
+        if (lane == 0) {
+            a.done[q] = d ? 1u : 0u;
+            if (!d && a.rest_q) a.rest_q[atomicAdd(a.rest_cnt, 1u)] = (uint32_t)q;
+        }
     }
     uint32_t rank, sb, pp;
-    const uint32_t kk = wave_topk<NS>(key, sbits, pos, a.k, sc_all + wave * 64u, lane, rank, sb, pp);
+    const uint32_t kk = wave_topk<NS>(key, sbits, pos, a.k, sc, lane, rank, sb, pp);
     uint32_t child;
     if (lane_beam) {
         uint32_t jj = 0;
@@ -181,16 +180,56 @@
     if (lane == 0) a.out_cnt[q] = kk;
 }
 
+template <int NS>
+__global__ void __launch_bounds__(256) k2_topk_wave(K2Args a) {
+    __shared__ uint2 sc_all[4 * 64];
+    const int lane = threadIdx.x & 63;
+    const uint32_t wave = __builtin_amdgcn_readfirstlane(threadIdx.x >> 6);
+    const uint32_t q32 = blockIdx.x * 4u + wave;
+    if (q32 >= a.nrows) return;
+    if (a.skip_done && a.skip_done[q32]) return;
+    k2_wave_query<NS>(a, q32, sc_all + wave * 64u, lane);
+}
+
+typedef const __attribute__((address_space(4))) uint32_t K2ArgWord;
+static_assert(sizeof(K2Args) % 4 == 0 && alignof(K2Args) <= 8 && std::is_trivially_copyable<K2Args>::value, "k2_wave_query_reload copies K2Args as 32-bit words");
+template <int NS>
+__device__ __forceinline__ void k2_wave_query_reload(K2ArgWord* wp, const uint32_t q32, uint2* sc, const int lane) {
+    constexpr int NW = (int)(sizeof(K2Args) / 4);
+    union { K2Args a; uint32_t w[NW]; } u;
+    asm volatile("" : "+s"(wp));
+#pragma unroll
+    for (int i = 0; i < NW; ++i) u.w[i] = wp[i];
+    k2_wave_query<NS>(u.a, q32, sc, lane);
+}
+
+template <int NS>
+__global__ void __launch_bounds__(256) k2_topk_list(K2Args a) {
+    __shared__ uint2 sc_all[4 * 64];
+    const int lane = threadIdx.x & 63;
+    const uint32_t wave = __builtin_amdgcn_readfirstlane(threadIdx.x >> 6);
+    const uint32_t n_waves = gridDim.x * 4u, nq = min(*a.rest_cnt, a.nrows);
+    for (uint32_t i = blockIdx.x * 4u + wave; i < nq; i += n_waves) {
+        const uint32_t q32 = __builtin_amdgcn_readfirstlane(a.rest_q[i]);
+        if (q32 < a.nrows) k2_wave_query_reload<NS>((K2ArgWord*)__builtin_amdgcn_kernarg_segment_ptr(), q32, sc_all + wave * 64u, lane);
+        wave_sync_lds();
+    }
+}
+
 size_t k2_max_k() { return (160 * 1024) / 8; }
 
 bool k2_wave_path(const LayerPlan& P) { return P.k <= 64 && P.cand_stride <= 64u * 32u; }
 
 void launch_k2_topk(const LayerDev& L, const LayerPlan& P, BeamDev prev, const uint32_t* cand_off,
                     const uint32_t* ncand, const float* cand, BeamDev out, hipStream_t s, uint32_t rank_limit, uint32_t limited_cands,
-                    uint32_t* done, const uint32_t* skip_done, const uint32_t* xok) {
+                    uint32_t* done, const uint32_t* skip_done, const uint32_t* xok, uint32_t* rest_q, uint32_t* rest_cnt) {
     if (P.nrows == 0) return;
     K2Args a;
-    a.p_val = prev.val; a.rank_limit = rank_limit; a.done = done; a.skip_done = skip_done; a.xok = xok;
+    a.p_val = prev.val; a.rank_limit = rank_limit; a.done = done; a.skip_done = skip_done; a.xok = xok; a.rest_q = rest_q; a.rest_cnt = rest_cnt;
+    if (rest_q && !rest_cnt) fail("k2: the list of unfinished queries needs its count");
+    bool list = rest_q && !done;
+    if (list && !skip_done) fail("k2: the list form also takes the done flags (one instantiation keeps the batch-sized grid)");
+    if (list && (rank_limit || !k2_wave_path(P))) fail("k2: the list form serves the last stage of a bound-pruned layer");
     if (done && !xok) fail("k2: bound pruning needs the per-query guard flags");
     a.mult = (P.pp.kind == PP_SIGMOID || P.pp.kind == PP_LP_HINGE) ? 1 : 0;
     if ((rank_limit || done || skip_done) && !k2_wave_path(P)) fail("k2: bound pruning needs the register top-k path");
@@ -201,21 +240,26 @@
     a.nrows = P.nrows; a.beam_in = P.beam_in; a.cand_stride = P.cand_stride; a.k = P.k; a.out_stride = out.stride;
     a.implicit_root = P.implicit_root;
     if (P.k == 0) fail("k2: only_topk / beam_size resolved to 0");
-    if (!rank_limit && !done && !skip_done && (P.k > k2_max_k() || (P.tune.k2_big_min_k > 0 && P.k >= (uint32_t)P.tune.k2_big_min_k))) {
+    if (!rank_limit && !done && !skip_done && !list && (P.k > k2_max_k() || (P.tune.k2_big_min_k > 0 && P.k >= (uint32_t)P.tune.k2_big_min_k))) {
         launch_k2_topk_big(L, P, prev, cand_off, ncand, cand, out.idx, out.val, out.cnt, out.stride, s);
         return;
     }
     if (k2_wave_path(P)) {
         const uint32_t ns = ((rank_limit ? std::min(P.cand_stride, std::max(1u, limited_cands)) : P.cand_stride) + 63u) / 64u;
-        const dim3 grid((P.nrows + 3u) / 4u), block(256);
-        if (ns <= 1) hipLaunchKernelGGL(k2_topk_wave<1>, grid, block, 0, s, a);
-        else if (ns <= 2) hipLaunchKernelGGL(k2_topk_wave<2>, grid, block, 0, s, a);
-        else if (ns <= 4) hipLaunchKernelGGL(k2_topk_wave<4>, grid, block, 0, s, a);
-        else if (ns <= 8) hipLaunchKernelGGL(k2_topk_wave<8>, grid, block, 0, s, a);
-        else if (ns <= 13) hipLaunchKernelGGL(k2_topk_wave<13>, grid, block, 0, s, a);
-        else if (ns <= 16) hipLaunchKernelGGL(k2_topk_wave<16>, grid, block, 0, s, a);
-        else if (ns <= 24) hipLaunchKernelGGL(k2_topk_wave<24>, grid, block, 0, s, a);
-        else hipLaunchKernelGGL(k2_topk_wave<32>, grid, block, 0, s, a);
+        if (ns > 13 && ns <= 16) list = false;
+        const dim3 grid(list ? std::min<uint32_t>((P.nrows + 3u) / 4u, 1024u) : (P.nrows + 3u) / 4u), block(256);
+#define XRL_K2_WAVE(NN) do { if (list) hipLaunchKernelGGL(k2_topk_list<NN>, grid, block, 0, s, a); else hipLaunchKernelGGL(k2_topk_wave<NN>, grid, block, 0, s, a); } while (0)
+#define XRL_K2_GRID(NN) hipLaunchKernelGGL(k2_topk_wave<NN>, grid, block, 0, s, a)
+        if (ns <= 1) XRL_K2_WAVE(1);
+        else if (ns <= 2) XRL_K2_WAVE(2);
+        else if (ns <= 4) XRL_K2_WAVE(4);
+        else if (ns <= 8) XRL_K2_WAVE(8);
+        else if (ns <= 13) XRL_K2_WAVE(13);
+        else if (ns <= 16) XRL_K2_GRID(16);
+        else if (ns <= 24) XRL_K2_WAVE(24);
+        else XRL_K2_WAVE(32);
+#undef XRL_K2_GRID
+#undef XRL_K2_WAVE
     } else if (P.k <= 64) {
         hipLaunchKernelGGL(k2_topk_reg, dim3(P.nrows), dim3(64), 0, s, a);
     } else {
diff --git a/pecos_amd/csrc/xrl_kernels.h b/pecos_amd/csrc/xrl_kernels.h
--- a/pecos_amd/csrc/xrl_kernels.h
+++ b/pecos_amd/csrc/xrl_kernels.h
@@ -40,11 +40,12 @@
 void launch_k0_prolongate(const LayerDev& L, const LayerPlan& P, const QueriesDev& X, BeamDev prev, uint32_t* cand_off,
                           uint32_t* ncand, void* items, hipStream_t s, uint32_t item_ranks = 0xFFFFFFFFu );
 void launch_k0b_remaining(const LayerDev& L, const LayerPlan& P, const QueriesDev& X, BeamDev prev, const uint32_t* cand_off, const uint32_t* done,
-                          uint32_t first_rank, void* items, uint32_t* n_items, hipStream_t s, uint32_t end_rank = 0xFFFFFFFFu);
+                          uint32_t first_rank, void* items, uint32_t* n_items, hipStream_t s, uint32_t end_rank = 0xFFFFFFFFu,
+                          const uint32_t* rest_q = nullptr, const uint32_t* rest_cnt = nullptr);
 bool k2_wave_path(const LayerPlan& P);
 size_t k0_item_bytes();
-void launch_k1(const LayerDev& L, const LayerPlan& P, const QueriesDev& X, const void* items, const uint32_t* n_items,
-               float* cand, int group, hipStream_t s);
+bool launch_k1(const LayerDev& L, const LayerPlan& P, const QueriesDev& X, const void* items, const uint32_t* n_items,
+               float* cand, int group, hipStream_t s, uint32_t list_grid = 0);
 void launch_sort_items(const LayerDev& L, uint64_t n_slots, const void* items, void* sorted, uint32_t* H,
                        uint32_t* start, hipStream_t s,
                        const uint32_t* n_dev = nullptr);
@@ -58,7 +59,8 @@
                     const uint32_t* ncand, const float* cand, BeamDev out, hipStream_t s,
                     uint32_t rank_limit = 0 , uint32_t limited_cands = 0 ,
                     uint32_t* done = nullptr , const uint32_t* skip_done = nullptr ,
-                    const uint32_t* xok = nullptr );
+                    const uint32_t* xok = nullptr ,
+                    uint32_t* rest_q = nullptr, uint32_t* rest_cnt = nullptr );
 constexpr int kStatsPerLayer = 8;
 void launch_stats(const LayerDev& L, const LayerPlan& P, const QueriesDev& X, BeamDev prev, const uint32_t* ncand, const void* items,
                   double* out8, hipStream_t s, uint64_t item_slots = 0 );
@@ -86,7 +88,8 @@
                          uint32_t seg_stride = 1, uint32_t seg_off = 0, uint32_t* err = nullptr);
 int k1_auto_group(const LayerDev& L, const Layer& host, int dense);
 bool k1t_serves(const LayerDev& L, const QueriesDev& X);
-struct K1TSelect { BeamDev prev; const uint32_t* xok; BeamDev out; uint32_t* done; uint32_t* cand_off; uint32_t* ncand; };
+struct K1TSelect { BeamDev prev; const uint32_t* xok; BeamDev out; uint32_t* done; uint32_t* cand_off; uint32_t* ncand;
+                   uint32_t* rest_q = nullptr; uint32_t* rest_cnt = nullptr; };
 bool k1t_selects(const LayerDev& L, const LayerPlan& P, const QueriesDev& X);
 void launch_k1t(const LayerDev& L, const LayerPlan& P, const QueriesDev& X, const void* items, const uint32_t* n_items, float* cand, hipStream_t s,
                 const K1TSelect* sel = nullptr);
diff --git a/pecos_amd/csrc/xrl_model.h b/pecos_amd/csrc/xrl_model.h
--- a/pecos_amd/csrc/xrl_model.h
+++ b/pecos_amd/csrc/xrl_model.h
@@ -116,6 +116,7 @@
     DevBuf blk_start, x_ok;
     DevBuf qperm, qsort_hist, qsort_start;
     DevBuf prune_done, prune_cnt;
+    DevBuf rest_q;
 };
 struct Workspace {
     LaneWs lane[2];
@@ -166,6 +167,7 @@
         int adaptive = 1;
         int presence = 1;
         int leaf_fuse = 1;
+        int leaf_tail = 1;
         int prune_mid = 1;
         int sort_rest = 1;
         int sort_rest_min = 32768;
diff --git a/pecos_amd/csrc/xrl_predict.cpp b/pecos_amd/csrc/xrl_predict.cpp
--- a/pecos_amd/csrc/xrl_predict.cpp
+++ b/pecos_amd/csrc/xrl_predict.cpp
@@ -35,6 +35,7 @@
     uint32_t stage_end[3]; int n_stage;
     bool fuse, fuse_k0;
     bool sorts_rest;
+    bool compact_rest;
 };
 
 struct Batch {
@@ -48,7 +49,7 @@
     uint64_t row0 = 0; uint32_t nrows = 0; hipStream_t S = nullptr;
     bool x_ok_done = false;
     BeamDev beam[2]{};
-    uint32_t *cand_off, *ncand, *sort_hist, *sort_start, *blk_start, *x_ok, *qperm, *qsort_hist, *qsort_start, *prune_done, *prune_cnt;
+    uint32_t *cand_off, *ncand, *sort_hist, *sort_start, *blk_start, *x_ok, *qperm, *qsort_hist, *qsort_start, *prune_done, *prune_cnt, *rest_q;
     float* cand; void *items, *items_sorted;
 
     void begin_batch(const LaneWs& lw, hipStream_t s, uint64_t r0, uint32_t n) {
@@ -57,7 +58,7 @@
         for (int i = 0; i < 2; ++i) beam[i] = BeamDev{u32(lw.beam_idx[i]), lw.beam_val[i].as<float>(), u32(lw.beam_cnt[i]), beam_stride};
         cand_off = u32(lw.cand_off); ncand = u32(lw.ncand); cand = lw.cand.as<float>(); items = lw.items.p; items_sorted = lw.items_sorted.p;
         sort_hist = u32(lw.sort_hist); sort_start = u32(lw.sort_start); blk_start = u32(lw.blk_start); x_ok = u32(lw.x_ok);
-        qperm = u32(lw.qperm); qsort_hist = u32(lw.qsort_hist); qsort_start = u32(lw.qsort_start); prune_done = u32(lw.prune_done); prune_cnt = u32(lw.prune_cnt);
+        qperm = u32(lw.qperm); qsort_hist = u32(lw.qsort_hist); qsort_start = u32(lw.qsort_start); prune_done = u32(lw.prune_done); prune_cnt = u32(lw.prune_cnt); rest_q = u32(lw.rest_q);
     }
     bool unstaged(size_t l) const { return l < (size_t)kFbLayers && fb.unstaged[l]; }
     LayerPlan make_plan(size_t l) const {
@@ -188,6 +189,7 @@
     r.stage_end[r.n_stage++] = beam_in;
     r.fuse = opt.leaf_fuse != 0 && r.J == 1 && !b.stats && k1t_selects(L.dev, P, b.X);
     r.fuse_k0 = r.fuse && opt.leaf_fuse != 2 && beam_in <= 32u;
+    r.compact_rest = opt.leaf_tail != 0 && r.n_stage == 2 && !b.stats;
     return r;
 }
 
@@ -197,7 +199,7 @@
     for (size_t l = 0; l < T; ++l) {
         bin_max = std::max(bin_max, b.shape[l].beam_in); cs_max = std::max(cs_max, b.shape[l].cand_stride); slots_max = std::max<uint64_t>(slots_max, nb * b.shape[l].beam_in * m.layers[l]->max_tiles_per_parent);
     }
-    size_t sorted = 0, hist = 0, starts = 0, x_ok = 0, done = 0, cnt = 0, qperm = 0, qhist = 0, qstarts = 0;
+    size_t sorted = 0, hist = 0, starts = 0, x_ok = 0, done = 0, cnt = 0, rest = 0, qperm = 0, qhist = 0, qstarts = 0;
     for (const uint64_t rows : {nb, n_rows % nb}) {
         for (size_t l = 0; l < T && rows; ++l) {
             const Route r = route_layer(b, l, rows); const Layer& L = *m.layers[l];
@@ -205,6 +207,7 @@
             if (r.mode != 0 || (b.opt.prune && r.sorts_rest)) { hist = std::max(hist, sort_hist_bytes(nb * b.shape[l].beam_in * L.max_tiles_per_parent, L.n_tiles)); starts = std::max(starts, ((size_t)L.n_tiles + 1) * 4); }
             if (starts || staged_tile) sorted = slots_max * k0_item_bytes();
             if (staged_tile || (r.kind == ROUTE_K1G && r.pruned)) { done = (size_t)nb * 4; cnt = 256; }
+            if (staged_tile && r.compact_rest) rest = (size_t)nb * 4;
             if (r.kind == ROUTE_K1G || staged_tile || (r.kind == ROUTE_K1Q && b.opt.prune && r.last + 1 < T)) x_ok = (size_t)nb * 4;
             const uint32_t nk = m.layers[r.last]->dev.n_parents;
             if (r.kind == ROUTE_K1Q && r.sorted_last) { qperm = (size_t)nb * 4; qhist = std::max(qhist, qsort_hist_bytes((uint32_t)nb, nk)); qstarts = std::max(qstarts, ((size_t)nk + 1) * 4); }
@@ -216,7 +219,7 @@
         lw.items.reserve(slots_max * k0_item_bytes());
         lw.cand_off.reserve(nb * bin_max * 4); lw.ncand.reserve(nb * 4); lw.cand.reserve(nb * (uint64_t)cs_max * 4);
         lw.items_sorted.reserve(sorted); lw.sort_hist.reserve(hist); lw.sort_start.reserve(starts); lw.blk_start.reserve(starts);
-        lw.x_ok.reserve(x_ok); lw.prune_done.reserve(done); lw.prune_cnt.reserve(cnt);
+        lw.x_ok.reserve(x_ok); lw.prune_done.reserve(done); lw.prune_cnt.reserve(cnt); lw.rest_q.reserve(rest);
         lw.qperm.reserve(qperm); lw.qsort_hist.reserve(qhist); lw.qsort_start.reserve(qstarts);
     }
     if (b.stats) m.ws->stats.reserve(T * kStatsPerLayer * sizeof(double));
@@ -304,15 +307,17 @@
     }
     const uint64_t slots_b = (uint64_t)nrows * (beam_in - J) * L.max_tiles_per_parent;
     b.need_x_ok();
+    uint32_t* const rest_q = r.compact_rest ? b.rest_q : nullptr; uint32_t* const rest_cnt = r.compact_rest ? b.prune_cnt + 1 : nullptr;
+    if (r.compact_rest) b.timed("rest_list", l, [&] { XRL_HIP(hipMemsetAsync(b.prune_cnt, 0, 8, S)); });
     if (!r.fuse_k0) b.timed("k0_prolongate", l, [&] { launch_k0_prolongate(L.dev, P, X, prev, b.cand_off, b.ncand, b.items, S, J); });
     if (b.lanes == 2 && b.k1_done) XRL_HIP(hipStreamWaitEvent(S, b.k1_done, 0));
     if (r.fuse) {
-        const K1TSelect sel{prev, b.x_ok, out, b.prune_done, b.cand_off, b.ncand};
+        const K1TSelect sel{prev, b.x_ok, out, b.prune_done, b.cand_off, b.ncand, rest_q, rest_cnt};
         b.timed("k1_sparse", l, [&] { launch_k1t(L.dev, P, X, r.fuse_k0 ? nullptr : b.items, nullptr, b.cand, S, &sel); });
     } else {
         LayerPlan PA = P; PA.beam_in = J;
         b.timed(k1_name[0], l, [&] { launch_k1(L.dev, PA, X, b.items, nullptr, b.cand, r.group, S); });
-        b.timed("k2_topk", l, [&] { launch_k2_topk(L.dev, P, prev, b.cand_off, b.ncand, b.cand, out, S, J, (uint32_t)L.cand_bound(J), b.prune_done, nullptr, b.x_ok); });
+        b.timed("k2_topk", l, [&] { launch_k2_topk(L.dev, P, prev, b.cand_off, b.ncand, b.cand, out, S, J, (uint32_t)L.cand_bound(J), b.prune_done, nullptr, b.x_ok, rest_q, rest_cnt); });
     }
     if (stats) XRL_HIP(hipMemsetAsync(b.items_sorted, 0xFF, slots_b * k0_item_bytes(), S));
     bool srt = r.sorts_rest;
@@ -325,11 +330,20 @@
     for (int st = 1; st < r.n_stage; ++st) {
         const uint32_t r0 = r.stage_end[st - 1], r1 = r.stage_end[st]; const bool last = st == r.n_stage - 1;
         LayerPlan PB = P; PB.beam_in = r1 - r0; PB.tune.wpb = 4;
-        b.timed(last ? "k0b_remaining" : "k0b_remaining_mid", l, [&] { launch_k0b_remaining(L.dev, P, X, prev, b.cand_off, b.prune_done, r0, srt ? b.items : b.items_sorted, b.prune_cnt, S, r1); });
+        uint32_t list_grid = 0; bool ran_list = false;
+        if (rest_q) {
+            const uint64_t slots_s = (uint64_t)nrows * (r1 - r0) * L.max_tiles_per_parent;
+            const uint32_t seen = P.fb_host ? m.fb.word(fb_items_word((int)l)) : kFbPending;
+            if (b.opt.leaf_tail >= 2) list_grid = (uint32_t)b.opt.leaf_tail;
+            else if (seen != kFbPending && slots_s >= (1ull << 21) && (uint64_t)seen * 8u <= slots_s) list_grid = 6144;
+        }
+        b.timed(last ? "k0b_remaining" : "k0b_remaining_mid", l, [&] { launch_k0b_remaining(L.dev, P, X, prev, b.cand_off, b.prune_done, r0, srt ? b.items : b.items_sorted, b.prune_cnt, S, r1, rest_q, rest_cnt); });
         if (srt) b.timed(last ? "k1_sort_items_rest" : "k1_sort_items_mid", l, [&] { launch_sort_items(L.dev, (uint64_t)nrows * (r1 - r0) * L.max_tiles_per_parent, b.items, b.items_sorted, b.sort_hist, b.sort_start, S, b.prune_cnt); });
-        b.timed(k1_name[last ? 2 : 1], l, [&] { launch_k1(L.dev, PB, X, b.items_sorted, srt ? b.sort_start + L.n_tiles : b.prune_cnt, b.cand, r.group, S); });
+        b.timed(k1_name[last ? 2 : 1], l, [&] { ran_list = launch_k1(L.dev, PB, X, b.items_sorted, srt ? b.sort_start + L.n_tiles : b.prune_cnt, b.cand, r.group, S, list_grid); });
+        if (ran_list && b.named()) b.timed("rest_list_grid", l, [] {});
         if (b.lanes == 2 && last) { b.k1_done = b.next_event(); XRL_HIP(hipEventRecord(b.k1_done, S)); }
-        if (last) b.timed("k2_topk_rest", l, [&] { launch_k2_topk(L.dev, P, prev, b.cand_off, b.ncand, b.cand, out, S, 0, 0, nullptr, b.prune_done); });
+        if (last && rest_q) b.timed("k2_topk_rest", l, [&] { launch_k2_topk(L.dev, P, prev, b.cand_off, b.ncand, b.cand, out, S, 0, 0, nullptr, b.prune_done, nullptr, rest_q, rest_cnt); });
+        else if (last) b.timed("k2_topk_rest", l, [&] { launch_k2_topk(L.dev, P, prev, b.cand_off, b.ncand, b.cand, out, S, 0, 0, nullptr, b.prune_done); });
         else b.timed("k2_topk_mid", l, [&] { launch_k2_topk(L.dev, P, prev, b.cand_off, b.ncand, b.cand, out, S, r1, (uint32_t)L.cand_bound(r1), b.prune_done, b.prune_done, b.x_ok); });
         if (stats && last) { launch_stats(L.dev, P, X, prev, b.ncand, b.items, stats, S, (uint64_t)nrows * J * L.max_tiles_per_parent); launch_stats(L.dev, PB, X, prev, nullptr, b.items_sorted, stats, S, slots_b); }
     }
```

After: 100.5 million queries/s (median of 6 runs). 1.03x the previous value.
